# Plachtaa/FAcodec

Measured on AMD Instinct MI355X. Metric: 24kHz audio sec encoded+decoded per wall-sec, higher is better.
Workload: dtype f32; 1 GPU; configs[1]: batch=32/GPU x 2 s @ 24 kHz, forward encoder->FVQ(6 codebooks)->decoder, FAcodec configs/config.yml model (137.7 M params), weights formula-generated, weight-norm re-materialised every step; clips_per_gpu=32, samples_per_clip=48000, parallelism=dp1 (independent clips, no collective)

## Files before the change

facodec_amd/_lib.py:

```python
import ctypes as C
import os

_HERE = os.path.dirname(os.path.abspath(__file__))
LIB_PATH = os.environ.get("FAC_LIB_PATH", os.path.join(_HERE, "libfacodec_hip.so"))

PAD_ZERO, PAD_REFLECT = 0, 1
ACT_NONE, ACT_TANH, ACT_MISH, ACT_LOG_MEL = 0, 1, 2, 3
ACT_GATE, ACT_WN_RES_SKIP = 4, 5

_p = C.c_void_p
_i = C.c_int
_i64 = C.c_int64
_f = C.c_float


class ConvDesc(C.Structure):
    _fields_ = [
        ("x", _p), ("w", _p), ("bias", _p), ("alpha_in", _p), ("alpha_out", _p), ("res", _p), ("y", _p), ("y2", _p), ("alpha_y2", _p), ("w_k1", _p), ("bias_k1", _p),
        ("x_bs", _i64), ("x_cs", _i64), ("y_bs", _i64), ("y_cs", _i64),
        ("B", C.c_int32), ("C_in", C.c_int32), ("T_in", C.c_int32), ("C_out", C.c_int32),
        ("C_out_pad", C.c_int32), ("T_out", C.c_int32),
        ("K", C.c_int32), ("stride", C.c_int32), ("dilation", C.c_int32), ("pad_left", C.c_int32),
        ("pad_mode", C.c_int32), ("n_phase", C.c_int32), ("y_tstride", C.c_int32), ("phase_shift", C.c_int32),
        ("act", C.c_int32),
        ("w_batched", C.c_int32), ("w_bs", _i64), ("ws", _p), ("ws_bytes", _i64), ("w_split", _p),
        ("K1", C.c_int32), ("dilation2", C.c_int32), ("row_phases", C.c_int32),
        ("x_p8", _p), ("x_p8_plane_bytes", _i64), ("y2_p8", _p), ("y2_p8_plane_bytes", _i64),
        ("pw_split", C.c_int32), ("split_rows", C.c_int32),
        ("gate_cond", _p), ("gate_cond_bs", _i64),
        ("keep_tile160", C.c_int32),
    ]


class VqDesc(C.Structure):
    _fields_ = [
        ("residual", _p), ("z_in", _p), ("zq_acc", _p), ("zq_out", _p), ("w_in", _p), ("b_in", _p),
        ("codebook", _p), ("w_out", _p), ("w_out_scale", _p), ("b_out", _p), ("mask", _p), ("codes", _p), ("z_e", _p),
        ("loss_part", _p), ("codes_bs", _i64),
        ("B", C.c_int32), ("D", C.c_int32), ("T", C.c_int32), ("Kc", C.c_int32),
    ]



VQ_DECODE_MAX_Q = 16


class VqDecodeDesc(C.Structure):
    _fields_ = [
        ("codes", _p * 3), ("codes_bs", _i64 * 3), ("codes_qs", _i64 * 3), ("n_q", C.c_int32 * 3),
        ("codebook", _p * VQ_DECODE_MAX_Q), ("w_out", _p * VQ_DECODE_MAX_Q), ("w_out_scale", _p * VQ_DECODE_MAX_Q),
        ("b_out", _p * VQ_DECODE_MAX_Q), ("style", _p), ("outs", _p), ("z", _p * 3),
        ("B", C.c_int32), ("D", C.c_int32), ("T", C.c_int32), ("Kc", C.c_int32),
    ]


class VqDecodeMaskedDesc(C.Structure):
    _fields_ = [("base", VqDecodeDesc), ("n_use", _p), ("n_use_bs", _i64), ("n_use_ts", _i64)]


PLC_MAX_FRAMES = 16
PLC_PRIMARY, PLC_REDUNDANT, PLC_LOST = 0, 1, 2


class PlcSelectDesc(C.Structure):
    _fields_ = [
        ("prim", _p * 3), ("prim_bs", _i64 * 3), ("prim_qs", _i64 * 3),
        ("red", _p * 3), ("red_bs", _i64 * 3), ("red_qs", _i64 * 3),
        ("dst", _p * 3), ("dst_bs", _i64 * 3), ("dst_qs", _i64 * 3),
        ("n_q", C.c_int32 * 3), ("n_red", C.c_int32 * 3),
        ("status", _p), ("last_codes", _p), ("last_n", _p), ("g", _p), ("run", _p),
        ("n_use", _p), ("n_use_bs", _i64), ("n_use_ts", _i64), ("ramp", _p),
        ("B", C.c_int32), ("k", C.c_int32), ("hold", C.c_int32), ("fade", C.c_int32), ("recover", C.c_int32),
        ("reserved", C.c_int32),
    ]


class CodesPackDesc(C.Structure):
    _fields_ = [
        ("codes", _p * 3), ("codes_bs", _i64 * 3), ("codes_qs", _i64 * 3), ("n_q", C.c_int32 * 3),
        ("lens", _p), ("out", _p), ("out_bs", _i64),
        ("B", C.c_int32), ("T", C.c_int32), ("bits", C.c_int32),
    ]


class CodesUnpackDesc(C.Structure):
    _fields_ = [
        ("in_", _p), ("in_bs", _i64), ("codes", _p * 3), ("codes_bs", _i64 * 3), ("codes_qs", _i64 * 3), ("n_q", C.c_int32 * 3),
        ("lens", _p),
        ("B", C.c_int32), ("T", C.c_int32), ("bits", C.c_int32),
    ]


class ResampleDesc(C.Structure):
    _fields_ = [
        ("hist", _p), ("x", _p), ("lens", _p), ("y", _p), ("hist_out", _p), ("table", _p), ("offs", _p),
        ("hist_bs", _i64), ("x_bs", _i64), ("y_bs", _i64), ("q0", _i64), ("m_lo", _i64),
        ("B", C.c_int32), ("n_hist", C.c_int32), ("T", C.c_int32), ("n_out", C.c_int32),
        ("o", C.c_int32), ("n", C.c_int32), ("taps", C.c_int32),
    ]


class KweightDesc(C.Structure):
    _fields_ = [
        ("x", _p), ("lens", _p), ("e", _p), ("state_in", _p), ("state_out", _p), ("peak", _p), ("ws", _p),
        ("x_bs", _i64), ("e_bs", _i64),
        ("B", C.c_int32), ("T", C.c_int32), ("S", C.c_int32), ("offset", C.c_int32), ("peak_accumulate", C.c_int32),
        ("reserved", C.c_int32),
        ("coef", C.c_double * 10), ("pw", C.c_double * 16 * 7),
    ]


SI_SDR_CHUNK = 4096


class StoiDesc(C.Structure):
    _fields_ = [
        ("x", _p), ("y", _p), ("lens", _p), ("kept_idx", _p), ("n_frames", _p), ("n_kept", _p), ("n_segments", _p),
        ("stoi", _p), ("estoi", _p), ("ws", _p),
        ("x_bs", _i64), ("y_bs", _i64), ("ws_bytes", _i64),
        ("B", C.c_int32), ("T", C.c_int32),
    ]


SLOT_MAX_DST, SLOT_TILE = 8, 4096


class SlotSeg(C.Structure):
    _fields_ = [
        ("base", _p), ("slot_hi", _i64),
        ("rows", C.c_int32), ("row_stride", C.c_int32), ("row_len", C.c_int32), ("slot_lo", C.c_int32),
        ("elems", C.c_int32), ("reserved", C.c_int32),
    ]


SIGNATURES = {
    "fac_version": (_i, []),
    "fac_last_error": (C.c_char_p, []),
    "fac_wn_scale": (_i, [_p, _p, _p, _i, _i, _p]),
    "fac_pack_conv_w": (_i, [_p, _p, _p, _i, _i, _i, _i, _p]),
    "fac_pack_convtr_w_rows": (_i, [_p, _p, _p, _i, _i, _i, _p]),
    "fac_conv_w_split_bytes": (_i64, [_i, _i, _i]),
    "fac_conv_w_split2_bytes": (_i64, [_i, _i, _i, _i]),
    "fac_pack_conv_w_split2": (_i, [_p, _p, _p, _i, _i, _i, _i, _p]),
    "fac_gemm_w_split_bytes": (_i64, [_i, _i, _i, _i]),
    "fac_pack_gemm_w_split": (_i, [_p, _i64, _i64, _i64, _p, _p, _i, _i, _i, _i, _p]),
    "fac_pack_conv_w_split": (_i, [_p, _p, _p, _i, _i, _i, _p]),
    "fac_conv_w_split_rows_bytes": (_i64, [_i, _i, _i, _i]),
    "fac_pack_conv_w_split_rows": (_i, [_p, _p, _p, _i, _i, _i, _i, _p]),
    "fac_flip_transpose_w": (_i, [_p, _p, _p, _i, _i, _i, _p]),
    "fac_prep_begin": (_i, []),
    "fac_prep_set_phase": (_i, [_i]),
    "fac_prep_abort": (_i, []),
    "fac_prep_end": (_i, []),
    "fac_prep_replay": (_i, [_i, _p]),
    "fac_prep_info": (_i, [_i, _p, _p]),
    "fac_prep_free": (_i, [_i]),
    "fac_pack_conv_w_bwd": (_i, [_p, _p, _p, _i, _i, _i, _i, _p]),
    "fac_pad_fold_bwd": (_i, [_p, _p, _i, _i, _i, _i, _i, _i, _p]),
    "fac_conv1d_bwd_weight_ws_bytes": (_i64, [_i, _i, _i, _i, _i]),
    "fac_conv1d_bwd_weight": (_i, [_p, _p, _p, _p, _i64, _i, _i, _i, _i, _i, _i, _i, _i, _i, _i, _i, _i, _p]),
    "fac_conv1d_bwd_weight_split_ws_bytes": (_i64, [_i, _i, _i, _i, _i, _i, _i, _i, _i, _i]),
    "fac_conv1d_bwd_weight_split_form": (_i, [_i, _i, _i, _i, _i, _i, _i, _i, _i, _i, _i, C.POINTER(C.c_int)]),
    "fac_conv1d_bwd_weight_k1_ws_bytes": (_i64, [_i, _i, _i, _i]),
    "fac_conv1d_bwd_weight_k1_ws_bytes_for": (_i64, [_p, _p, _i, _i, _i, _i]),
    "fac_conv1d_bwd_weight_taps_tx": (_i64, [_i, _i, _i, _i, _i]),
    "fac_conv1d_bwd_weight_taps_ws_bytes": (_i64, [_i, _i, _i, _i, _i, _i, _i, _i]),
    "fac_conv1d_bwd_weight_taps_ws_bytes_for": (_i64, [_p, _i, _i, _i, _i, _i, _i, _i, _i]),
    "fac_conv1d_bwd_weight_taps": (_i, [_p, _p, _p, _p, _p, _i64, _i, _i, _i, _i, _i, _i, _i, _i, _i, _p]),
    "fac_conv1d_bwd_weight_k1": (_i, [_p, _p, _p, _p, _p, _i64, _i, _i, _i, _i, _p]),
    "fac_conv1d_bwd_weight_split": (_i, [_p, _p, _p, _p, _i64, _i, _i, _i, _i, _i, _i, _i, _i, _i, _i, _i, _i, _p]),
    "fac_conv1d_bwd_weight_split_db_ok": (_i, [_i, _i, _i, _i, _i, _i, _i, _i, _i, _i]),
    "fac_conv1d_bwd_weight_split_db": (_i, [_p, _p, _p, _p, _p, _i64, _i, _i, _i, _i, _i, _i, _i, _i, _i, _i, _i, _i, _p]),
    "fac_weight_norm_bwd": (_i, [_p, _p, _p, _p, _p, _i, _i, _p]),
    "fac_snake_bwd": (_i, [_p, _p, _p, _p, _p, _p, _i, _i, _i, _p]),
    "fac_pack_lstm_whh_t": (_i, [_p, _p, _i, _p]),
    "fac_lstm_layer_bwd": (_i, [_p, _p, _p, _p, _p, _p, _i, _i, _i, _p]),
    "fac_to_p8": (_i, [_p, _p, _p, _i, _i, _i, _p]),
    "fac_lstm_persist_ok": (_i, [_i, _i]),
    "fac_lstm_persist_stream_ok": (_i, [_p]),
    "fac_pack_lstm_whh16": (_i, [_p, _p, _i, _i, _p]),
    "fac_lstm_layer_fwd_persist": (_i, [_p, _p, _p, _p, _p, _p, _i, _i, _i, _i, _p]),
    "fac_lstm_layer_bwd_persist": (_i, [_p, _p, _p, _p, _p, _p, _i, _i, _i, _i, _p]),
    "fac_lstm_persist_split_ok": (_i, [_i, _i]),
    "fac_lstm_persist_timeouts": (_i, []),
    "fac_lstm_persist_arm": (_i, [_p]),
    "fac_lstm_abort_flag": (_i, [_p, _p]),
    "fac_mask_flags_if": (_i, [_p, _i, _p, _p]),
    "fac_pack_lstm_whh_split": (_i, [_p, _p, _i, _p]),
    "fac_lstm_layer_fwd_persist_split": (_i, [_p, _p, _p, _p, _i, _i, _i, _i, _p]),
    "fac_snake_bwd_fused": (_i, [_p, _p, _p, _p, _p, _p, _p, _p, _i, _i, _i, _p]),
    "fac_bias_grad": (_i, [_p, _p, _p, _i, _i, _i, _p]),
    "fac_snake_bwd_fused_rs": (_i, [_p, _p, _p, _i64, _p, _p, _p, _p, _p, _i, _i, _i, _p]),
    "fac_pad_fold_edges": (_i, [_p, _i, _i, _i, _i, _i, _p]),
    "fac_pack_convtr_w": (_i, [_p, _p, _p, _i, _i, _i, _i, _p]),
    "fac_conv1d_fwd": (_i, [C.POINTER(ConvDesc), _p]),
    "fac_conv1d_variant": (_i, [C.POINTER(ConvDesc), C.c_char_p, _i]),
    "fac_snake_fwd": (_i, [_p, _p, _p, _i, _i, _i, _p]),
    "fac_lstm_to_time_major": (_i, [_p, _p, _i, _i, _i, _p]),
    "fac_lstm_from_time_major": (_i, [_p, _p, _p, _p, _i, _i, _i, _p]),
    "fac_pack_lstm_whh": (_i, [_p, _p, _i, _p]),
    "fac_lstm_layer_fwd": (_i, [_p, _p, _p, _p, _i, _i, _i, _p]),
    "fac_lstm_layer_fwd_from": (_i, [_p, _p, _p, _p, _i, _i, _i, _i64, _p]),
    "fac_lstm_layer_fwd_train": (_i, [_p, _p, _p, _p, _p, _p, _i, _i, _i, _i64, _p]),
    "fac_lstm_gate_bwd": (_i, [_p, _p, _p, _p, _p, _p, _p, _i, _i, _i64, _i, _p]),
    "fac_tanh_bwd": (_i, [_p, _p, _p, _i64, _p]),
    "fac_pair_bwd": (_i, [_p, _p, _p, _i64, _i, C.c_float, C.c_float, _i, _p]),
    "fac_spec_power_bwd": (_i, [_p, _p, _p, _i, _i, _i, _i, _p]),
    "fac_stft_frames_bwd": (_i, [_p, _p, _i, _i, _i, _i, _i, _i, _i, _p]),
    "fac_vq_latent_bwd": (_i, [_p, _p, _p, _i64, _p, _p, _p, _p, _i, _i, _p]),
    "fac_vq_codebook_grad": (_i, [_p, _p, _p, _i64, _p, _p, _i, _i, _i, _i, _p]),
    "fac_layernorm_c_affine_bwd": (_i, [_p, _p, _p, _p, _p, _p, _i, _i, _i, _p]),
    "fac_rows_fma": (_i, [_p, _p, _p, _p, _i, _i64, _f, _p]),
    "fac_grad_norm_clip": (_i, [_p, _i64, _f, _p, _p, _p]),
    "fac_adamw_step": (_i, [_p, _p, _p, _p, _i64, _f, _f, _f, _f, _f, _i64, _p, _p]),
    "fac_logdiff_rms_bwd": (_i, [_p, _p, _p, _i, _i, _i, _f, _f, _i, _p]),
    "fac_gather_copy": (_i, [_p, _p, _p, _i, _p]),
    "fac_adamw_step_masked": (_i, [_p, _p, _p, _p, _i64, _p, _i, _p, _p, _p, _f, _f, _f, _f, _f, _p, _p]),
    "fac_gate_bwd": (_i, [_p, _p, _p, _i, _i, _i, _p]),
    "fac_mish_fwd": (_i, [_p, _p, _i64, _p]),
    "fac_mish_bwd": (_i, [_p, _p, _p, _i64, _p]),
    "fac_glu_bwd": (_i, [_p, _p, _p, _i, _i, _i, _p]),
    "fac_mul_scaled": (_i, [_p, _p, _p, _f, _i64, _p]),
    "fac_embed_sum_bwd": (_i, [_p, _p, _p, _i, _i, _i, _i, _i, _i, _i, _p]),
    "fac_gate_bwd_cond": (_i, [_p, _p, _i64, _p, _p, _p, _i64, _i, _i, _i, _p]),
    "fac_masked_mean_bwd": (_i, [_p, _p, _p, _i, _i, _i, _p]),
    "fac_attention_probs": (_i, [_p, _p, _p, _p, _i, _i, _i, _i, _p]),
    "fac_attention_pv": (_i, [_p, _p, _p, _i, _i, _i, _i, _p]),
    "fac_attention_bwd_pv": (_i, [_p, _p, _p, _p, _p, _i, _i, _i, _i, _p]),
    "fac_attention_bwd_qk": (_i, [_p, _p, _p, _p, _p, _p, _p, _i, _i, _i, _i, _p]),
    "fac_aa_snakebeta_bwd": (_i, [_p, _p, _p, _p, _p, _p, _p, _p, _p, _i, _i, _i, _p]),
    "fac_leaky_relu": (_i, [_p, _p, _p, _i64, _f, _i, _i, _i, _i, _i, _p]),
# ... 107 lines not shown
```

facodec_amd/build.py:

```python
import os
import subprocess
import sys
from concurrent.futures import ThreadPoolExecutor

HERE = os.path.dirname(os.path.abspath(__file__))
CSRC = os.path.join(HERE, "csrc")
TAG = os.environ.get("FAC_BUILD_TAG", "")
LIB = os.path.join(HERE, "libfacodec_hip%s.so" % ("_" + TAG if TAG else ""))
OBJDIR = "build" + ("_" + TAG if TAG else "")
SOURCES = ["conv1d_api.hip", "conv1d_tile_128x128.hip", "conv1d_tile_96x128.hip", "conv1d_tile_64x128.hip",
           "conv1d_tile_32x256.hip", "conv1d_tile_128x32.hip", "conv1d_tile_128x256.hip", "conv1d_fused_ru.hip", "conv1d_narrow.hip", "conv1d_pw.hip", "conv1d_pw_split.hip", "conv1d_skinny.hip", "conv1d_bsplit.hip", "conv1d_bsplit96.hip", "conv1d_gemm_split.hip", "conv1d_bsplit2.hip", "conv1d_bwd.hip", "conv1d_wgrad_split.hip", "conv1d_wgrad_k1.hip", "train_misc.hip", "optim.hip", "train_quant.hip", "train_pred.hip", "train_disc.hip", "train_redecoder.hip", "pack.hip", "prep_batch.hip", "lstm.hip", "lstm_persist.hip", "vq.hip", "vq_decode.hip", "bitpack.hip", "misc.hip", "attention_stream.hip", "attention_tiled.hip","ragged.hip", "resample.hip", "loudness.hip", "metrics.hip", "stream_pool.hip", "plc.hip", "jdc.hip", "rccl_arena.hip"]
FLAGS = ["--offload-arch=gfx950", "-O3", "-std=c++17", "-fPIC", "-ffp-contract=off",
         "-Wno-unused-result"] + os.environ.get("FAC_EXTRA_FLAGS", "").split()


def _hipcc():
    for cand in (os.environ.get("HIPCC"), "/opt/rocm/bin/hipcc", "hipcc"):
        if cand and (os.path.isabs(cand) and os.path.exists(cand) or not os.path.isabs(cand)):
            return cand
    return "hipcc"


def _stale(target, deps):
    if not os.path.exists(target):
        return True
    tt = os.path.getmtime(target)
    return any(os.path.getmtime(d) > tt for d in deps)


def build_lib(force=False, verbose=True):
    hipcc = _hipcc()
    headers = sorted(os.path.join(CSRC, f) for f in os.listdir(CSRC) if f.endswith(".h")) + [os.path.join(HERE, "..", "include", "facodec_hip.h")]
    objs, jobs = [], []
    os.makedirs(os.path.join(CSRC, OBJDIR), exist_ok=True)
    for src in SOURCES:
        s = os.path.join(CSRC, src)
        o = os.path.join(CSRC, OBJDIR, src.replace(".hip", ".o"))
        objs.append(o)
        if force or _stale(o, [s] + headers):
            jobs.append([hipcc, *FLAGS, "-c", s, "-o", o])

    def run(cmd):
        if verbose:
            print(" ".join(cmd), file=sys.stderr)
        subprocess.run(cmd, check=True)

    with ThreadPoolExecutor(max_workers=min(8, max(1, len(jobs)))) as ex:
        list(ex.map(run, jobs))
    if force or jobs or _stale(LIB, objs):
        run([hipcc, "--offload-arch=gfx950", "-shared", "-fPIC", *objs, "-ldl", "-o", LIB])
    return LIB


if __name__ == "__main__":
    build_lib(force="--force" in sys.argv)
    print(LIB)
```

facodec_amd/convplan.py:

```python
from collections import namedtuple

__all__ = ["ConvPlan", "ConvTrPlan", "plan_conv", "plan_convtr", "plan_gemm", "tile_rows", "gemm_split_ok", "gemm_split_strided_ok", "split2_ok",
           "pw_taps_ok", "pw_split_tail_ok", "convtr_split_ok", "convtr_rows_ok", "flat_strided_ok", "flat_convtr_ok", "W_FP32", "W_TAPS",
           "W_GEMM", "W_GEMM_STRIDED", "W_SPLIT2", "W_FP32_PW_TAPS", "PER_CLIP", "FLAT_STRIDED", "FLAT_STRIDE1", "TR_POLYPHASE", "TR_ROWS",
           "TR_ROWS_SPLIT", "TR_ROWS_PW_TAPS", "TR_FLAT"]

W_FP32, W_TAPS, W_GEMM, W_GEMM_STRIDED, W_SPLIT2, W_FP32_PW_TAPS = "fp32", "split_taps", "split_gemm", "split_gemm_strided", "split2", "fp32_pw_taps"
PER_CLIP, FLAT_STRIDED, FLAT_STRIDE1 = "per_clip", "flat_strided", "flat_stride1"
ConvPlan = namedtuple("ConvPlan", "layout form p8")
TR_POLYPHASE, TR_ROWS, TR_ROWS_SPLIT, TR_ROWS_PW_TAPS, TR_FLAT = "polyphase", "rows", "rows_split", "rows_pw_taps", "flat_rows_split"
ConvTrPlan = namedtuple("ConvTrPlan", "layout p8")


def _sw():
    from . import ops
    return ops


def gemm_split_ok(c_out, c_in, k, n_cols, t_out=None):
    sw = _sw()
    if not (sw.BF16_SPLIT and k in (1, 2)):
        return False
    if c_in < sw.GEMM_SPLIT_MIN_CIN or c_out < 64 or n_cols < 1024:
        return False
    return k == 1 or (t_out is not None and t_out >= 256)


def gemm_split_strided_ok(c_out, c_in, k, stride, batch, t_out):
    return (_sw().BF16_SPLIT and 1 < stride <= 16 and stride < k <= 2 * stride and c_in >= 32
            and c_out >= 64 and t_out >= 256 and batch * t_out >= 1024)


def split2_ok(c_out, k, k1, stride, n_cols):
    kv = k1 if 0 < k1 < k else k
    return (_sw().BF16_SPLIT and 8 <= c_out <= 32 and ((kv == 9 and stride in (1, 2)) or (kv == 3 and stride == 1))
            and n_cols >= 4096)


def pw_split_tail_ok(c_in, c_out, cols):
    sw = _sw()
    return sw.BF16_SPLIT and sw.PW_SPLIT and c_in == c_out and c_in in (256, 384) and cols >= 65536


def pw_taps_ok(c_in, c_out, k, stride, transposed, batch, t_out):
    sw = _sw()
    if not (sw.BF16_SPLIT and sw.PW_SPLIT and sw.PW_TAPS and stride == 2):
        return False
    taps, rows = (2, 2 * c_out) if transposed else (4, c_out)
    if k != 4 or (c_in * taps) % 64 or c_in * taps > 384 or rows % 64:
        return False
    return batch * ((t_out + 31) // 32) >= 2 * (256 // (rows // 64)) * 12


def convtr_rows_ok(t_in, stride, causal=True):
    sw = _sw()
    return sw.CONVTR_ROWS and causal and 2 <= stride <= 16 and t_in >= sw.CONVTR_ROWS_MIN_T


def convtr_split_ok(c_in, c_out, stride, batch, t_in, causal=True, alpha_in=None):
    return (_sw().BF16_SPLIT and causal and alpha_in is None and 2 <= stride <= 16 and c_in >= 64
            and t_in >= 256 and batch * t_in >= 1024 and c_out * stride >= 64)


def flat_strided_ok(c_out, c_in, k, s, batch, n_out):
    return (_sw().FLAT_TRAIN and k == 2 * s and s > 1 and n_out < 256 and not gemm_split_strided_ok(c_out, c_in, k, s, batch, n_out)
            and gemm_split_strided_ok(c_out, c_in, k, s, 1, batch * (n_out + 1) - 1))


def flat_convtr_ok(c_in, c_out, s, batch, t_cols):
    return (_sw().FLAT_TRAIN and t_cols < 256 and not convtr_split_ok(c_in, c_out, s, batch, t_cols)
            and convtr_split_ok(c_in, c_out, s, 1, batch * t_cols))


def tile_rows(c_out, c_in, k, grad=False):
    sw = _sw()
    return 96 if (sw.BF16_SPLIT and not grad and k == 7 and c_out in sw.BS_ROWS96 and c_in % 8 == 0) else 64


def plan_conv(c_out, c_in, k, stride, dilation, batch, t_in, t_out, *, k1=0, alpha_in=False, plain=True, res=False,
              causal_reflect=False, grad=True, c_out_mult16=True, split_k=(1, 3, 5, 7), floor_k=(3, 5), tail="pw_split",
              pw_taps=True, split2=False, flat_infer=False, flat_stride1=False, flat_train=None):
    sw = _sw()
    cols = batch * t_out
    p8 = 2.0 * c_out * k / (4.0 * stride)
    if split2 and split2_ok(c_out, k, k1, stride, cols):
        return ConvPlan(W_SPLIT2, PER_CLIP, None)
    if stride > 1:
        strided = not alpha_in and dilation == 1 and not k1
        flat_t = (flat_train is not None and strided and plain and t_in % stride == 0
                  and (flat_train == "zero" or (causal_reflect and t_in > stride))
                  and flat_strided_ok(c_out, c_in, k, stride, batch, t_out))
        if flat_t and flat_train == "reflect":
            return ConvPlan(W_GEMM_STRIDED, FLAT_STRIDED, p8)
        if pw_taps and stride == 2 and strided and plain and pw_taps_ok(c_in, c_out, k, 2, False, batch, t_out):
            return ConvPlan(W_FP32_PW_TAPS, PER_CLIP, None)
        if strided and gemm_split_strided_ok(c_out, c_in, k, stride, batch, t_out):
            return ConvPlan(W_GEMM_STRIDED, PER_CLIP, p8)
        if flat_t:
            return ConvPlan(W_GEMM_STRIDED, FLAT_STRIDED, p8)
        if (flat_infer and strided and not res and causal_reflect and k == 2 * stride and t_in % stride == 0 and t_in > stride
                and not grad and gemm_split_strided_ok(c_out, c_in, k, stride, 1, batch * (t_in // stride + 1) - 1)):
            return ConvPlan(W_GEMM_STRIDED, FLAT_STRIDED, p8)
    elif not alpha_in and not k1 and k in split_k:
        if k == 1 and gemm_split_ok(c_out, c_in, 1, cols):
            if not (pw_split_tail_ok(c_in, c_out, cols) if tail == "pw_split"
                    else tail is not None and c_in == c_out and c_in in (256, 384) and cols >= 65536):
                return ConvPlan(W_GEMM, PER_CLIP, None)
        if (sw.BF16_SPLIT and k in (3, 5, 7) and c_in % 16 == 0 and c_out > 2 and (c_out % 16 == 0 or not c_out_mult16)
                and cols > 640 and (k not in floor_k or (c_in >= 64 and c_out > 32))):
            if (flat_infer and flat_stride1 and k == 7 and not res and causal_reflect and not grad and batch >= 4
                    and (k - 1) * dilation < t_in <= 224 and c_in * c_out >= 1 << 20):
                return ConvPlan(W_TAPS, FLAT_STRIDE1, None)
            return ConvPlan(W_TAPS, PER_CLIP, None)
    return ConvPlan(W_FP32, PER_CLIP, None)


def plan_gemm(c_out, c_in, n_cols):
    ok = gemm_split_ok(c_out, c_in, 1, n_cols)
    return ConvPlan(W_GEMM if ok else W_FP32, PER_CLIP, 2.0 * c_out / 4.0 if ok else None)


def plan_convtr(c_in, c_out, stride, batch, t_in, *, causal=True, alpha_in=False, grad=True, flat_infer=False, flat_train_cols=None):
    a = True if alpha_in else None
    p8 = 2.0 * c_out * 2 * stride / 4.0
    if causal and flat_train_cols is not None and flat_convtr_ok(c_in, c_out, stride, batch, flat_train_cols):
        return ConvTrPlan(TR_FLAT, p8)
    if causal and not alpha_in and pw_taps_ok(c_in, c_out, 2 * stride, stride, True, batch, t_in):
        return ConvTrPlan(TR_ROWS_PW_TAPS, None)
    if convtr_split_ok(c_in, c_out, stride, batch, t_in, causal, a):
        return ConvTrPlan(TR_ROWS_SPLIT, p8)
    if flat_infer and not grad and t_in < 256 and convtr_split_ok(c_in, c_out, stride, 1, batch * (t_in + 1), causal, a):
        return ConvTrPlan(TR_FLAT, p8)
    return ConvTrPlan(TR_ROWS if convtr_rows_ok(t_in, stride, causal) else TR_POLYPHASE, None)
```

facodec_amd/csrc/conv1d_api.hip:

```cpp
#include "conv1d_mfma.h"
#include <stdlib.h>

namespace fac {

enum ConvKernel : int {
  CK_128x32 = 0,
  CK_32x256 = 1,
  CK_64x128 = 2,
  CK_96x128 = 3,
  CK_128x128 = 4,
  CK_128x256 = 5,
  CK_96x256 = 6,
  CK_FUSED_RU = 7,
  CK_128x160 = 8,
  CK_NARROW = 9,
  CK_SKINNY = 10,
  CK_BSPLIT = 11,
  CK_CIN1 = 12,
  CK_THIN = 13,
  CK_PW = 14,
  CK_GSPLIT = 15,
  CK_BSPLIT2 = 16,
  CK_PWS = 17,
  CK_PWT = 18,
  CK_BSPLIT96 = 19,
};

static ConvKernel select_variant(const fac_conv_desc* d) {
  const int co = d->C_out;
  if (d->row_phases > 1) return CK_128x256;
  if (d->T_out <= 32) return CK_128x32;
  if (co <= 32) return CK_32x256;
  if (co <= 64) return CK_64x128;
  const bool wide = d->K == 1 && d->n_phase == 1 && d->T_out >= 512;
  if (d->T_out > 128 && d->T_out <= 160 && co > 64) {
    const long long wide_tiles = (long long)d->B * ((co + 127) / 128);
    if (d->K == 1 && d->stride == 1 && d->n_phase == 1 && !d->keep_tile160 && wide_tiles < 256) return CK_128x32;
    return CK_128x160;
  }
  if (co % 128 != 0 && co % 96 == 0) return wide ? CK_96x256 : CK_96x128;
  return wide ? CK_128x256 : CK_128x128;
}

static bool narrow_ok(const fac_conv_desc* d) {
  return d->C_out <= 2 && d->stride == 1 && d->n_phase == 1 && d->phase_shift == 0 && d->y_tstride == 1 && !d->res && !d->y2 &&
         !d->w_batched && d->y && (long long)d->B <= 65535 && (long long)d->B * ((d->T_out + 1023) / 1024) >= 128;
}

static bool pw_enabled() {
  static const bool on = !(getenv("FAC_PW") && getenv("FAC_PW")[0] == '0');
  return on;
}

static int conv_plan(const fac_conv_desc* d, ConvArgs& a, ConvKernel& k) {
  FAC_REQUIRE(d && (d->x || d->x_p8) && (d->w || d->w_split) && (d->y || d->y2 || d->y2_p8), "conv1d: null pointer");
  FAC_REQUIRE(!d->y2 || d->alpha_y2 || d->act == FAC_ACT_WN_RES_SKIP, "conv1d: y2 needs alpha_y2");
  FAC_REQUIRE(d->B > 0 && d->C_in > 0 && d->C_out > 0 && d->T_in > 0 && d->T_out > 0,
              "conv1d: bad shape B=%d C_in=%d C_out=%d T_in=%d T_out=%d", d->B, d->C_in, d->C_out,
              d->T_in, d->T_out);
  FAC_REQUIRE(d->K >= 1 && d->stride >= 1 && d->dilation >= 1 && d->pad_left >= 0,
              "conv1d: bad K/stride/dilation/pad");
  FAC_REQUIRE(d->C_out_pad % 32 == 0 && (d->C_out_pad >= d->C_out || d->row_phases > 1), "conv1d: C_out_pad must be a multiple of 32");
  FAC_REQUIRE(d->n_phase >= 1 && d->y_tstride >= 1, "conv1d: bad phase config");
  FAC_REQUIRE((long long)d->B * d->n_phase <= 65535, "conv1d: B*n_phase too large for grid.z");
  a.x = d->x; a.w = d->w; a.bias = d->bias; a.alpha_in = d->alpha_in; a.alpha_out = d->alpha_out;
  a.res = d->res; a.y = d->y; a.y2 = d->y2; a.alpha2 = d->alpha_y2;
  a.w1 = d->w_k1; a.bias1 = d->bias_k1;
  a.x_p8 = reinterpret_cast<const unsigned char*>(d->x_p8); a.x_p8_ps = d->x_p8_plane_bytes;
  a.y2_p8 = reinterpret_cast<unsigned char*>(d->y2_p8); a.y2_p8_ps = d->y2_p8_plane_bytes;
  FAC_REQUIRE(!d->y2_p8 || d->alpha_y2, "conv1d: y2_p8 needs alpha_y2");
  if (d->w_k1) {
    FAC_REQUIRE(d->C_in == d->C_out && d->C_out_pad == d->C_out && d->n_phase == 1 && d->stride == 1 &&
                    d->alpha_out && d->act == FAC_ACT_NONE && !d->w_batched,
                "conv1d: fused ResidualUnit needs C_in == C_out (multiple of 32), stride 1, a Snake alpha_out");
  }
  a.x_bs = d->x_bs; a.x_cs = d->x_cs; a.y_bs = d->y_bs; a.y_cs = d->y_cs; a.w_bs = d->w_bs;
  a.B = d->B; a.C_in = d->C_in; a.T_in = d->T_in; a.C_out = d->C_out; a.C_out_pad = d->C_out_pad;
  a.T_out = d->T_out; a.K = d->K; a.stride = d->stride; a.dil = d->dilation;
  a.pad_left = d->pad_left; a.pad_mode = d->pad_mode; a.n_phase = d->n_phase;
  a.y_tstride = d->y_tstride; a.act = d->act; a.w_batched = d->w_batched;
  a.phase_shift = d->phase_shift;
  a.rp = d->row_phases > 1 ? d->row_phases : 1;
  FAC_REQUIRE(!d->gate_cond || (d->act == FAC_ACT_GATE && d->gate_cond_bs >= 0),
              "conv1d: gate_cond is the conditioning row of the FAC_ACT_GATE epilogue (act=%d gate_cond_bs=%lld)", d->act,
              (long long)d->gate_cond_bs);
  a.gate_cond = d->gate_cond; a.gate_cond_bs = d->gate_cond_bs;
  if (a.rp > 1) {
    FAC_REQUIRE(d->n_phase == 1 && d->y_tstride == 1 && d->phase_shift == 0 && d->stride == 1 && a.rp <= 128 && !d->w_k1 &&
                    !d->w_batched && d->C_out_pad == fac_convtr_rows(d->C_out, a.rp) && !(d->K1 > 0 && d->K1 < d->K),
                "conv1d: row_phases needs a plain stride-1 launch on weights from fac_pack_convtr_w_rows");
  }
  a.K1 = d->K1 > 0 ? d->K1 : d->K; a.dil2 = d->dilation2;
  FAC_REQUIRE(a.K1 <= d->K && d->K % a.K1 == 0 && (a.K1 == d->K || d->dilation2 > 0), "conv1d: bad two-level taps (K=%d K1=%d)", d->K, d->K1);
  FAC_REQUIRE(!conv_two_level(a) || (!d->w_k1 && d->n_phase == 1 && d->pad_mode == FAC_PAD_ZERO && !d->w_batched),
              "conv1d: two-level taps need a plain, zero-padded conv");
  conv_set_virtual(a);
  FAC_REQUIRE(d->phase_shift >= 0 && d->phase_shift < d->n_phase + (d->n_phase == 1), "conv1d: bad phase_shift");
  {
    long long last = (long long)(d->T_out - 1) * d->stride + (long long)conv_max_tap_offset(a) - d->pad_left;
    int pad_right = last >= d->T_in ? (int)(last - d->T_in + 1) : 0;
    int max_pad = d->pad_left > pad_right ? d->pad_left : pad_right;
    a.T_ext = d->T_in > max_pad ? d->T_in : max_pad + 1;
  }
  if (d->x_p8 || d->y2_p8) {
    const bool gs = d->w_split && (d->K <= 2 || (d->stride > 1 && d->K <= 2 * d->stride)) && conv_gsplit_ok(a) &&
                    !conv_skinny_ok(a, d->ws, d->ws_bytes) && d->C_in % 8 == 0 && d->x_p8_plane_bytes < (1ll << 32);
    const bool ok = !d->y2_p8 && (gs || (d->w_split && !conv_two_level(a) && (d->split_rows == 96 ? conv_bsplit96_p8_ok(a) : conv_bsplit_p8_ok(a)) &&
                                       !conv_cin1_ok(a)));
    FAC_REQUIRE(ok, "conv1d: P8 operands given but the launch does not run on a kernel that takes them (K=%d stride=%d C_in=%d columns=%lld)",
                d->K, d->stride, d->C_in, (long long)d->B * d->T_out);
  }
  if (d->act == FAC_ACT_GATE || d->act == FAC_ACT_WN_RES_SKIP) {
    FAC_REQUIRE(d->w && !d->w_k1 && !d->x_p8 && !conv_two_level(a) && conv_skinny_ok(a, d->ws, d->ws_bytes),
                "conv1d: FAC_ACT_GATE / FAC_ACT_WN_RES_SKIP exist only for few-column launches (B * T_out <= 640) with a workspace");
    k = CK_SKINNY;
    return FAC_OK;
  }
  if (d->w_k1) { k = CK_FUSED_RU; return FAC_OK; }
  a.gflat = 0;
  a.grt = 0;
  if (d->w_split && (a.KV == 9 || a.KV == 3) && d->C_out <= 32 && conv_bsplit2_ok(a)) {
    a.w = reinterpret_cast<const float*>(d->w_split);
    k = CK_BSPLIT2;
    return FAC_OK;
  }
  FAC_REQUIRE(!conv_two_level(a) || d->w, "conv1d: two-level taps outside the split kernel's shapes need fp32 weights");
  const bool pw_on = pw_enabled();
  if (pw_on && d->pw_split && d->w && conv_pwt_ok(a)) { k = CK_PWT; return FAC_OK; }
  if (d->w_split && (d->K <= 2 || (d->stride > 1 && d->K <= 2 * d->stride)) && conv_gsplit_ok(a) &&
      !conv_skinny_ok(a, d->ws, d->ws_bytes)) {
    a.w = reinterpret_cast<const float*>(d->w_split);
    k = CK_GSPLIT;
    return FAC_OK;
  }
  if (a.rp > 1) {
    FAC_REQUIRE(d->w != nullptr && d->w != (const float*)d->w_split, "conv1d: row_phases launch outside the split kernel's shapes needs fp32 weights");
    k = CK_128x256;
    return FAC_OK;
  }
  const bool two_level = conv_two_level(a);
  FAC_REQUIRE(d->split_rows == 0 || d->split_rows == 64 || d->split_rows == 96, "conv1d: split_rows must be 0, 64 or 96");
  if (d->split_rows == 96) {
    FAC_REQUIRE(d->w_split && !two_level && conv_bsplit96_ok(a) && !conv_cin1_ok(a),
                "conv1d: split_rows = 96 needs a stride-1 k = 7 launch with C_out %% 96 == 0, C_in %% 8 == 0 and more than 640 columns "
                "(K=%d stride=%d C_in=%d C_out=%d columns=%lld)", d->K, d->stride, d->C_in, d->C_out, (long long)d->B * d->T_out);
    a.w = reinterpret_cast<const float*>(d->w_split);
    k = CK_BSPLIT96;
    return FAC_OK;
  }
  if (d->w_split && !two_level && conv_bsplit_ok(a) && !conv_cin1_ok(a)) {
    a.w = reinterpret_cast<const float*>(d->w_split);
    k = CK_BSPLIT;
    return FAC_OK;
  }
  FAC_REQUIRE(d->w != nullptr && (const void*)d->w != d->w_split,
              "conv1d: shape does not qualify for a split-bf16 kernel (K=%d stride=%d C_in=%d C_out=%d columns=%lld) and no fp32 "
              "weights were given", d->K, d->stride, d->C_in, d->C_out, (long long)d->B * d->T_out);
  if (!two_level && conv_skinny_ok(a, d->ws, d->ws_bytes)) k = CK_SKINNY;
  else if (narrow_ok(d) && (!two_level || (a.KV - 1) * a.dil <= 64)) k = CK_NARROW;
  else if (conv_thin_ok(a, d->ws, d->ws_bytes)) k = CK_THIN;
  else if (conv_cin1_ok(a)) k = CK_CIN1;
  else if (pw_on && d->pw_split && conv_pw_ok(a) && conv_pws_ok(a)) k = CK_PWS;
  else if (pw_on && conv_pw_ok(a)) k = CK_PW;
  else k = select_variant(d);
  return FAC_OK;
}

}

extern "C" int fac_conv1d_fwd(const fac_conv_desc* d, fac_stream_t stream) {
  using namespace fac;
  ConvArgs a;
  ConvKernel k;
  if (const int rc = conv_plan(d, a, k)) return rc;
  hipStream_t s = (hipStream_t)stream;
  switch (k) {
    case CK_128x32: return conv_dispatch_128x32(a, s);
    case CK_32x256: return conv_dispatch_32x256(a, s);
    case CK_64x128: return conv_dispatch_64x128(a, s);
    case CK_96x128: return conv_dispatch_96x128(a, s);
    case CK_128x128: return conv_dispatch_128x128(a, s);
    case CK_128x256: return conv_dispatch_128x256(a, s);
    case CK_96x256: return conv_dispatch_96x256(a, s);
    case CK_FUSED_RU: return conv_dispatch_fused_ru(a, s);
    case CK_128x160: return conv_dispatch_128x160(a, s);
    case CK_NARROW: return conv_dispatch_narrow(a, s);
    case CK_SKINNY: return conv_dispatch_skinny(a, d->ws, d->ws_bytes, s);
    case CK_BSPLIT: return conv_dispatch_bsplit(a, s);
    case CK_CIN1: return conv_dispatch_cin1(a, s);
    case CK_THIN: return conv_dispatch_thin(a, d->ws, s);
    case CK_PW: return conv_dispatch_pw(a, s);
    case CK_GSPLIT: return conv_dispatch_gsplit(a, s);
    case CK_BSPLIT2: return conv_dispatch_bsplit2(a, s);
    case CK_PWS: return conv_dispatch_pws(a, s);
    case CK_PWT: return conv_dispatch_pwt(a, s);
    case CK_BSPLIT96: return conv_dispatch_bsplit96(a, s);
  }
  return FAC_ERR_ARG;
}

extern "C" int fac_conv1d_variant(const fac_conv_desc* d, char* name, int name_len) {
  using namespace fac;
  ConvArgs a;
  ConvKernel k;
  if (const int rc = conv_plan(d, a, k)) return rc;
  if (!name || name_len <= 0) return k;
  switch (k) {
    case CK_128x32: snprintf(name, name_len, "conv1d_mfma_kernel<1,1,4,1,K> 128x32"); break;
    case CK_32x256: snprintf(name, name_len, "conv1d_mfma_kernel<1,2,1,4,K> 32x256"); break;
    case CK_64x128: snprintf(name, name_len, "conv1d_mfma_kernel<2,1,1,4,K> 64x128"); break;
    case CK_96x128: snprintf(name, name_len, "conv1d_mfma_kernel<3,1,1,4,K> 96x128"); break;
    case CK_128x128: snprintf(name, name_len, "conv1d_mfma_kernel<2,2,2,2,K> 128x128"); break;
    case CK_128x256:
      snprintf(name, name_len, a.rp > 1 ? "conv1d_mfma_kernel<2,2,2,4,2> 128x256 (convtr, all phases per tile)" : "conv1d_mfma_kernel<2,2,2,4,K> 128x256");
      break;
    case CK_96x256: snprintf(name, name_len, "conv1d_mfma_kernel<3,1,1,8,K> 96x256"); break;
    case CK_FUSED_RU: snprintf(name, name_len, "conv1d_mfma_kernel<C/32,1,1,4,7,fused RU> Cx128"); break;
    case CK_128x160: snprintf(name, name_len, "conv1d_mfma_kernel<1,5,4,1,K> 128x160"); break;
    case CK_NARROW:
      snprintf(name, name_len, conv_two_level(a) ? "conv1d_narrow_kernel (VALU, C_out<=2, two-level taps)" : "conv1d_narrow_kernel (VALU, C_out<=2)");
      break;
    case CK_SKINNY:
      snprintf(name, name_len, conv_skinny_single_launch(a) ? "conv1d_gemv_kernel (single launch, <=4 columns)"
                                                            : "conv1d_skinny_kernel (split reduction, <=640 columns)");
      break;
    case CK_BSPLIT: snprintf(name, name_len, "conv1d_bsplit_kernel<%d> 64x256 (bf16x3 split, fp32-grade)", a.K); break;
    case CK_CIN1: snprintf(name, name_len, "conv1d_cin1_kernel (VALU, C_in=1, store stream)"); break;
    case CK_THIN: snprintf(name, name_len, "conv1d_thin_kernel (VALU, C_out<=8, split channels)"); break;
    case CK_PW: snprintf(name, name_len, "conv1d_pw_kernel (k=1 streaming, W in LDS)"); break;
    case CK_GSPLIT:
      snprintf(name, name_len, "conv1d_gemm_split_kernel<%d> 128x128 (bf16x3 split GEMM, fp32-grade)", a.stride > 1 ? 2 : a.K);
      break;
    case CK_BSPLIT2: snprintf(name, name_len, "conv1d_bsplit2_kernel<%d,%d> 32x512 (bf16x3 split, fp32-grade)", a.KV, a.stride); break;
    case CK_PWS: snprintf(name, name_len, "conv1d_pws_kernel (k=1 streaming, W planes in LDS, bf16x3 split, fp32-grade)"); break;
    case CK_PWT: snprintf(name, name_len, "conv1d_pwt_kernel<%d taps> (streaming, W planes in LDS, bf16x3 split, fp32-grade)", a.K); break;
    case CK_BSPLIT96: snprintf(name, name_len, "conv1d_bsplit_kernel<%d> 96x256 (bf16x3 split, fp32-grade)", a.K); break;
  }
  return k;
}
```

facodec_amd/csrc/conv1d_bsplit_kernel.h:

```cpp
#pragma once
#include "conv1d_mfma.h"
#include <type_traits>
#include "inflight_regs.h"
#include "prep_batch.h"

namespace fac {

constexpr int BS_CO = 64;
constexpr int BS96_CO = 96;
constexpr int BS_NSW = 4;
constexpr int BS_NSW_WIDE = 4;
constexpr int BS_XU = 3;
constexpr int BS_WIDE_MIN = 64;
__host__ __device__ constexpr int bs_group(int C_in) { return C_in >= BS_WIDE_MIN ? 2 : 1; }

__host__ __device__ constexpr int bs_slots(int K, int G) { return (G * K + 1) & ~1; }

struct EpiRow {
  float bs, al, inv, a2, i2;
};
__device__ __forceinline__ EpiRow epi_row_load(bool valid, int co, const float* bias, const float* alpha, const float* alpha2) {
  EpiRow r = {0.f, 0.f, 0.f, 0.f, 0.f};
  if (valid) {
    if (bias) r.bs = bias[co];
    if (alpha) { r.al = alpha[co]; r.inv = snake_inv(r.al); }
    if (alpha2) { r.a2 = alpha2[co]; r.i2 = snake_inv(r.a2); }
  }
  return r;
}
__device__ __forceinline__ float epi_row_get(float mine, int lane, int j) {
  return __int_as_float(__builtin_amdgcn_ds_bpermute(((lane & 48) + j) << 2, __float_as_int(mine)));
}

template <int KT, int G, int NMW, int NSW, int MB = 2>
__global__ __launch_bounds__((NMW + NSW) * 64, (NMW + NSW) / 4) void conv1d_bsplit_kernel(ConvArgs a) {
  constexpr int NB = 2;
  constexpr int CO = 32 * MB;
  constexpr bool WIDE = NMW == 4;
  constexpr int BS_TT = 64 * NMW;
  constexpr int H = bs_slots(KT, G);
  constexpr int W_STAGE = 3 * H * CO * 16;
  extern __shared__ __attribute__((aligned(16))) unsigned char sm[];
  const int tid = threadIdx.x;
  const int lane = tid & 63;
  const int wave = __builtin_amdgcn_readfirstlane(tid >> 6);
  const int XW = a.XW;
  const int X_STAGE = 48 * G * XW;
  const int STG = W_STAGE + X_STAGE;
  unsigned char* Wbuf = sm;
  unsigned char* Xbuf = sm + W_STAGE;
  const int n_chunks = (a.C_in + 8 * G - 1) / (8 * G);
  const int dil = a.dil;

  const int n_tiles = a.n_tiles;
  typedef const __attribute__((address_space(4))) ConvArgs* KArgP;
  const KArgP kargs = (KArgP)__builtin_amdgcn_kernarg_segment_ptr();
  auto fresh_args = [&]() {
    KArgP q = kargs;
    asm volatile("" : "+s"(q));
    return q;
  };
  auto decode = [&](KArgP ka, int v, int& t0_, int& co0_, int& b_) {
    const int id = xcd_contiguous_id(v, n_tiles);
    const int nt = ka->n_t_tiles;
    const int tt = id % nt;
    const int rest = id / nt;
    const int nb = ka->B;
    b_ = rest % nb;
    co0_ = (rest / nb) * CO;
    t0_ = tt * BS_TT;
  };
  const bool overlap = a.persist != 0;
  unsigned char* epi_base = sm + (overlap ? STG : 0);
  auto walk = [&](auto role) {
  constexpr int ROLE = decltype(role)::value;
  constexpr bool STAGING = ROLE != 0;
  bool first = true;
  unsigned cboff[BS_XU] = {}, nboff[BS_XU] = {};
  unsigned long long cmask[BS_XU] = {}, nmask[BS_XU] = {};
  const float *cxg = nullptr, *nxg = nullptr;
  const unsigned char *cws = nullptr, *nws = nullptr;
  for (int vb = blockIdx.x; vb < n_tiles; vb += gridDim.x) {
  int t0, co0, b;
  decode(fresh_args(), vb, t0, co0, b);
  const bool has_nt = overlap && vb + (int)gridDim.x < n_tiles;

  if constexpr (STAGING) {
    const int lw = wave - NMW;
    __builtin_amdgcn_s_setprio(FAC_PRIO_STAGE);
    const float* xg = a.x + (long long)b * a.x_bs;
    const int xcs = (int)a.x_cs;
    const unsigned char* wsrc = reinterpret_cast<const unsigned char*>(a.w) + (long long)(co0 / CO) * n_chunks * W_STAGE;
    const int n_blk = (XW + 63) >> 6;
    int u_g[BS_XU], u_c[BS_XU], u_idx[BS_XU];
#pragma unroll
    for (int j = 0; j < BS_XU; ++j) {
      const int u = lw + NSW * j;
      u_g[j] = u % G;
      const int c = (u / G) * 64 + lane;
      u_c[j] = (u < G * n_blk && c < XW) ? c : -1;
      const int tin = t0 - a.pad_left + c;
      int idx;
      if (a.pad_mode == FAC_PAD_REFLECT) idx = reflect_index(tin, a.T_in, a.T_ext);
      else idx = (tin >= 0 && tin < a.T_in) ? tin : -1;
      u_idx[j] = u_c[j] >= 0 ? idx : -1;
    }
    constexpr int NBLK = W_STAGE / 1024;
    constexpr int ND = (NBLK + NSW - 1) / NSW;
    constexpr int NX = BS_XU * 8;
    static_assert(W_STAGE % 1024 == 0 && ND + NX <= 63 && NX == 24, "vmcnt is a 6-bit counter; FAC_XREGS24_* list 24 registers per set");
    auto stage_w = [&](int chunk, int buf) {
      constexpr int N16 = W_STAGE / 16;
      const unsigned char* src = wsrc + (long long)chunk * W_STAGE;
      unsigned char* dst = Wbuf + buf * STG;
      for (int i = lw; i * 64 < N16; i += NSW) {
        const int q = i * 64 + lane;
        if (q < N16)
          __builtin_amdgcn_global_load_lds((glb_void_t*)(src + (long long)q * 16), (lds_void_t*)(dst + i * 1024), 16, 0, 0);
      }
    };
    auto write_x = [&](int buf, const float (&xr)[BS_XU][8]) {
      unsigned char* xd = Xbuf + buf * STG;
#pragma unroll
      for (int j = 0; j < BS_XU; ++j) {
        if (u_c[j] < 0) continue;
        bf16x8 h, m, l;
#pragma unroll
        for (int i = 0; i < 8; ++i) {
          __bf16 p0, p1, p2;
          split3_scalar_sub(xr[j][i], p0, p1, p2);
          h[i] = p0; m[i] = p1; l[i] = p2;
        }
        *reinterpret_cast<bf16x8*>(xd + ((0 * G + u_g[j]) * XW + u_c[j]) * 16) = h;
        *reinterpret_cast<bf16x8*>(xd + ((1 * G + u_g[j]) * XW + u_c[j]) * 16) = m;
        *reinterpret_cast<bf16x8*>(xd + ((2 * G + u_g[j]) * XW + u_c[j]) * 16) = l;
      }
    };
    if constexpr (ROLE == 2) {
      typedef float wv4 __attribute__((ext_vector_type(4)));
      const unsigned char* xp = a.x_p8 + (long long)b * (a.C_in / 8) * a.T_in * 16;
      const long long grp_bytes = (long long)a.T_in * 16;
      unsigned u_poff[BS_XU];
      bool any_pad = false;
#pragma unroll
      for (int j = 0; j < BS_XU; ++j) {
        u_poff[j] = (unsigned)(u_idx[j] >= 0 ? u_idx[j] : 0) * 16u;
        any_pad = any_pad || __builtin_amdgcn_ballot_w64(u_c[j] >= 0 && u_idx[j] < 0) != 0;
      }
      for (int c = -1; c < n_chunks; ++c) {
        if (c + 1 < n_chunks) {
          const int buf = (c + 1) & 1;
          wv4 wv[ND], xv[BS_XU][3];
          const unsigned char* src = wsrc + (long long)(c + 1) * W_STAGE;
#pragma unroll
          for (int j = 0; j < ND; ++j) {
            const int bi = min(lw + NSW * j, NBLK - 1);
// ... 231 lines not shown
            __builtin_amdgcn_sched_barrier(0);
          } else {
            asm volatile("s_waitcnt lgkmcnt(0)" ::: "memory");
            __builtin_amdgcn_s_barrier();
            asm volatile("" ::: "memory");
            __builtin_amdgcn_sched_barrier(0);
            if (chunk + 1 < n_chunks) {
              if (cur == 0) ld(buf ^ 1, 0, A[1], Bf[1]); else ld(buf ^ 1, 0, A[0], Bf[0]);
            }
            if (cur == 0) mma(A[0], Bf[0]); else mma(A[1], Bf[1]);
            if (chunk + 1 < n_chunks) interleave();
            __builtin_amdgcn_sched_barrier(0);
          }
        }
      }
    }
    };
    if (MB == 2 && co0 + 32 >= a.C_out) pipeline(std::integral_constant<int, 1>{});
    else pipeline(std::integral_constant<int, MB>{});
  } else {
  for (int chunk = 0; chunk < n_chunks; ++chunk) {
    const int buf = chunk & 1;
    const unsigned char* Wb = Wbuf + buf * STG + (kq * CO + l31) * 16;
    const unsigned char* Xb = Xbuf + buf * STG + (n0 + l31) * 16 + x_lane;
    bf16x8 A[2][MB][3], Bf[1][NB][3];
    auto ldA = [&](int st, bf16x8 (&Ad)[MB][3]) {
#pragma unroll
      for (int p = 0; p < 3; ++p)
#pragma unroll
        for (int m = 0; m < MB; ++m)
          Ad[m][p] = *reinterpret_cast<const bf16x8*>(Wb + ((p * H + 2 * st) * CO + m * 32) * 16);
    };
    auto ldB = [&](int st, bf16x8 (&Bd)[NB][3]) {
      const int xo = st * x_step;
      constexpr int PO[3] = {1, 0, 2};
#pragma unroll
      for (int pi = 0; pi < 3; ++pi)
#pragma unroll
        for (int n = 0; n < NB; ++n)
          Bd[n][PO[pi]] = *reinterpret_cast<const bf16x8*>(Xb + xo + (PO[pi] * G * XW + n * 32) * 16);
    };
#pragma unroll
    for (int st = 0; st < H / 2; ++st) {
      ldB(st, Bf[0]);
      ldA(st, A[0]);
      __builtin_amdgcn_sched_barrier(0);
      constexpr int TA[6] = {1, 2, 0, 1, 0, 0}, TB[6] = {1, 0, 2, 0, 1, 0};
#pragma unroll
      for (int q = 0; q < 6; ++q)
#pragma unroll
        for (int m = 0; m < MB; ++m)
#pragma unroll
          for (int n = 0; n < NB; ++n)
            acc[m][n] = __builtin_amdgcn_mfma_f32_32x32x16_bf16(A[0][m][TA[q]], Bf[0][n][TB[q]], acc[m][n], 0, 0, 0);
      __builtin_amdgcn_sched_barrier(0);
    }
    __syncthreads();
  }
  }
  __builtin_amdgcn_s_setprio(0);
  {
    float* tile = reinterpret_cast<float*>(epi_base);
    constexpr int EP = BS_TT + 4;
    if constexpr (MB == 3) {
      int lane_off = 4 * kq * EP + n0 + l31;
      asm volatile("" : "+v"(lane_off));
      tile += lane_off;
#pragma unroll
      for (int m = 0; m < MB; ++m)
#pragma unroll
        for (int n = 0; n < NB; ++n)
#pragma unroll
          for (int r = 0; r < 16; ++r) tile[(m * 32 + (r & 3) + 8 * (r >> 2)) * EP + n * 32] = acc[m][n][r];
    } else
#pragma unroll
    for (int m = 0; m < MB; ++m)
#pragma unroll
      for (int n = 0; n < NB; ++n)
#pragma unroll
        for (int r = 0; r < 16; ++r)
          tile[(m * 32 + (r & 3) + 8 * (r >> 2) + 4 * kq) * EP + n0 + n * 32 + l31] = acc[m][n][r];
  }
  }
  __syncthreads();

  {
    const KArgP e = fresh_args();
    const float* tile = reinterpret_cast<const float*>(epi_base);
    constexpr int EP = BS_TT + 4;
    constexpr int NTH = (NMW + NSW) * 64;
    constexpr int QPR = BS_TT / 4;
    float* yg = e->y ? e->y + (long long)b * e->y_bs : nullptr;
    float* y2g = e->y2 ? e->y2 + (long long)b * e->y_bs : nullptr;
    const float* rg = e->res ? e->res + (long long)b * e->y_bs : nullptr;
    const bool vec_ok = (e->y_cs & 3) == 0 && (e->y_bs & 3) == 0 && (!yg || (reinterpret_cast<unsigned long long>(e->y) & 15) == 0) &&
                        (!y2g || (reinterpret_cast<unsigned long long>(e->y2) & 15) == 0) &&
                        (!rg || (reinterpret_cast<unsigned long long>(e->res) & 15) == 0);
    static_assert(QPR % 16 == 0 && NTH % 16 == 0 && (CO * QPR) % 64 == 0 && (CO * QPR + NTH - 1) / NTH <= 16, "EpiRow: 16 lanes share a row, <= 16 iterations");
    const int row_l = (tid + NTH * (lane & 15)) / QPR;
    const EpiRow mine = epi_row_load(row_l < CO && co0 + row_l < e->C_out, co0 + row_l, e->bias, e->alpha_out, y2g ? e->alpha2 : nullptr);
    int j = 0;
    for (int q = tid; q < CO * QPR; q += NTH, ++j) {
      const float bs = epi_row_get(mine.bs, lane, j), al = epi_row_get(mine.al, lane, j), inv = epi_row_get(mine.inv, lane, j);
      float a2 = 0.f, i2 = 0.f;
      if (y2g) { a2 = epi_row_get(mine.a2, lane, j); i2 = epi_row_get(mine.i2, lane, j); }
      const int row = q / QPR, tq = q - row * QPR;
      const int co = co0 + row, t = t0 + 4 * tq;
      if (co >= e->C_out || t >= e->T_out) continue;
      const float4 av = *reinterpret_cast<const float4*>(tile + row * EP + 4 * tq);
      f32x2 v[2] = {{av.x, av.y}, {av.z, av.w}};
      const long long o = (long long)co * e->y_cs + t;
      const bool full = vec_ok && t + 3 < e->T_out;
      float rv[4] = {0.f, 0.f, 0.f, 0.f};
      if (rg) {
        if (full) {
          const float4 r4 = *reinterpret_cast<const float4*>(rg + o);
          rv[0] = r4.x; rv[1] = r4.y; rv[2] = r4.z; rv[3] = r4.w;
        } else {
#pragma unroll
          for (int i = 0; i < 4; ++i) rv[i] = t + i < e->T_out ? rg[o + i] : 0.f;
        }
      }
#pragma unroll
      for (int i = 0; i < 2; ++i) {
        f32x2 x = v[i] + bs;
        if (e->alpha_out) x = snake_apply2(x, al, inv);
        if (e->act != FAC_ACT_NONE) { x.x = apply_act_slow(x.x, e->act); x.y = apply_act_slow(x.y, e->act); }
        v[i] = x + (f32x2){rv[2 * i], rv[2 * i + 1]};
      }
      f32x2 w[2] = {};
      if (y2g) {
#pragma unroll
        for (int i = 0; i < 2; ++i) w[i] = snake_apply2(v[i], a2, i2);
      }
      if (full) {
        if (yg) *reinterpret_cast<float4*>(yg + o) = make_float4(v[0].x, v[0].y, v[1].x, v[1].y);
        if (y2g) *reinterpret_cast<float4*>(y2g + o) = make_float4(w[0].x, w[0].y, w[1].x, w[1].y);
      } else {
#pragma unroll
        for (int i = 0; i < 4; ++i) {
          if (t + i >= e->T_out) continue;
          if (yg) yg[o + i] = v[i >> 1][i & 1];
          if (y2g) y2g[o + i] = w[i >> 1][i & 1];
        }
      }
    }
  }
  first = !overlap;
  if (vb + (int)gridDim.x < n_tiles) __syncthreads();
  }
  };
  if (wave >= NMW) {
    if constexpr (WIDE) {
      if (a.x_p8 != nullptr) walk(std::integral_constant<int, 2>{});
      else walk(std::integral_constant<int, 1>{});
    } else {
      walk(std::integral_constant<int, 1>{});
    }
  } else {
    walk(std::integral_constant<int, 0>{});
  }
}

template <int KT, int G, int NMW, int NSW, int MB = 2>
static int bsplit_launch(ConvArgs& a, hipStream_t s) {
  constexpr int H = bs_slots(KT, G), TT = 64 * NMW, CO = 32 * MB;
  a.XW = TT + (H / G - 1) * a.dil;
  const size_t stg = (size_t)3 * H * CO * 16 + (size_t)48 * G * a.XW;
  const size_t epi = (size_t)CO * (TT + 4) * sizeof(float);
  a.n_t_tiles = (a.T_out + TT - 1) / TT;
  const long long n_wg = (long long)a.n_t_tiles * ((a.C_out + CO - 1) / CO) * a.B;
  if (n_wg > 0x7fffffffll) {
    set_error("conv1d: too many workgroups (%lld)", n_wg);
    return FAC_ERR_ARG;
  }
  const int n_chunks = (a.C_in + 8 * G - 1) / (8 * G);
  int cus = device_cus() & ~7;
  a.persist = (NMW == 4 && a.x_p8 == nullptr && n_chunks % 2 == 0 && cus >= 8 && n_wg > cus &&
               stg + (stg > epi ? stg : epi) <= FAC_LDS_MAX) ? 1 : 0;
  size_t lds = a.persist ? stg + (stg > epi ? stg : epi) : (2 * stg > epi ? 2 * stg : epi);
  if (lds > FAC_LDS_MAX) {
    set_error("conv1d(bf16 split): tile needs %zu B of LDS (dil=%d)", lds, a.dil);
    return FAC_ERR_ARG;
  }
  constexpr auto kern = conv1d_bsplit_kernel<KT, G, NMW, NSW, MB>;
  allow_dynamic_lds<kern>();
  a.n_tiles = (int)n_wg;
  hipLaunchKernelGGL(kern, dim3((unsigned)(a.persist ? cus : n_wg)), dim3((NMW + NSW) * 64), lds, s, a);
  return check_launch("conv1d_bsplit");
}

}
```

facodec_amd/csrc/conv1d_mfma.h:

```cpp
#pragma once
#include "common.h"

namespace fac {

typedef __attribute__((address_space(3))) void lds_void_t;
typedef __attribute__((address_space(1))) const void glb_void_t;

constexpr int CONV_XMAX = 6;

struct ConvArgs {
  const float* x;
  const float* w;
  const float* bias;
  const float* alpha_in;
  const float* alpha_out;
  const float* res;
  float* y;
  float* y2;
  const float* alpha2;
  const float* w1;
  const float* bias1;
  long long x_bs, x_cs, y_bs, y_cs, w_bs;
  int B, C_in, T_in, T_ext, C_out, C_out_pad, T_out;
  int K, stride, dil, pad_left, pad_mode;
  int n_phase, y_tstride, act, w_batched;
  int phase_shift;
  int K1, dil2;
  int K2v, KV, CV;
  int cic;
  int XW;
  int XB;
  int XQ, XR;
  int n_t_tiles;
  int n_tiles, persist;
  int x_off;
  int gflat;
  int grt;
  const unsigned char* x_p8;
  long long x_p8_ps;
  unsigned char* y2_p8;
  long long y2_p8_ps;
  int rp;
  const float* gate_cond;
  long long gate_cond_bs;
};

__host__ __device__ inline int conv_max_tap_offset(const ConvArgs& a) {
  const int K1 = (a.K1 > 0 && a.K1 < a.K) ? a.K1 : a.K;
  return (a.K / K1 - 1) * a.dil2 + (K1 - 1) * a.dil;
}
__host__ __device__ inline bool conv_two_level(const ConvArgs& a) { return a.K1 > 0 && a.K1 < a.K; }
inline void conv_set_virtual(ConvArgs& a) {
  a.KV = conv_two_level(a) ? a.K1 : a.K;
  a.K2v = a.K / a.KV;
  a.CV = a.C_in * a.K2v;
}

template <int KT>
struct ConvUnroll {
  static constexpr int UC = (KT == 1) ? 4 : ((KT == 2 || KT == 3) ? 2 : 1);
  static constexpr int CIC = KT == 1 ? 24 : (KT == 2 || KT == 3) ? 16 : (KT >= 4 && KT <= 7) ? 8 : (KT > 7 ? 4 : 0);
};

template <int KT, int T_TILE>
constexpr int conv_cic() {
  return ((KT == 2 || KT == 3) && T_TILE >= 256) ? 8 : ConvUnroll<KT>::CIC;
}

constexpr int CONV_WPE = 4;
template <int MB, int NB, int WM, int WN, int KT, bool FUSE = false>
__global__ __launch_bounds__((WM * WN + 4) * 64, (WM * WN == 4 ? CONV_WPE : 3)) void conv1d_mfma_kernel(ConvArgs a) {
  constexpr int NMW = WM * WN;
  constexpr int CO_TILE = 32 * MB * WM;
  constexpr int T_TILE = 32 * NB * WN;
  constexpr int CO4 = CO_TILE / 4;
  constexpr bool ALLW = (WM * WN == 8) && !FUSE;
  extern __shared__ __attribute__((aligned(16))) float smem[];

  const int tid = threadIdx.x;
  const int lane = tid & 63;
  const int wave = __builtin_amdgcn_readfirstlane(tid >> 6);

  int t0, co0, b, phase;
  {
    const int id = xcd_contiguous_id<unsigned>(blockIdx.x, gridDim.x);
    const int nt = a.n_t_tiles, nbp = a.B * a.n_phase;
    const int tt = id % nt;
    const int rest = id / nt;
    const int bp = rest % nbp;
    const int ct = rest / nbp;
    t0 = tt * T_TILE;
    co0 = ct * CO_TILE;
    b = bp / a.n_phase;
    phase = bp - b * a.n_phase;
  }
  int y_off = phase - a.phase_shift, tap_shift = 0;
  if (y_off < 0) {
    y_off += a.n_phase;
    tap_shift = 1;
  }

  const int K = KT > 0 ? KT : a.KV;
  const int cic = KT > 0 ? conv_cic<KT, T_TILE>() : a.cic;
  const int XW = a.XW, XB = a.XB;
  const int w_stage = cic * K * CO_TILE;
  const int x_stage = cic * XW;
  float* Wbuf = smem;
  float* Xbuf = smem + 2 * w_stage;
  const int n_chunks = (a.CV + cic - 1) / cic;

  if (wave >= NMW) {
    const int lw = wave - NMW;
    __builtin_amdgcn_s_setprio(3);
    const float* xg = a.x + (long long)b * a.x_bs;
    const int w_rows_total = cin_pad_dev(a.C_in) * a.K;
    const float* wg = a.w + (long long)phase * w_rows_total * a.C_out_pad +
                      (a.w_batched ? (long long)b * a.w_bs : 0ll);
    const int tin0 = t0 * a.stride - a.pad_left - a.x_off;
    const bool vec_ok = ((a.x_cs | a.x_bs) & 3) == 0 && ((reinterpret_cast<unsigned long long>(a.x) & 15) == 0);
    const int r_first = lw / XB, cb_first = lw - r_first * XB;
    const int K2v = a.K2v, dil2 = a.dil2;
    const bool x_dma = a.alpha_in == nullptr && vec_ok && tin0 >= 0 && tin0 + (K2v - 1) * dil2 + XW <= a.T_in &&
                       (K2v == 1 || (dil2 & 3) == 0);

    auto stage = [&](int chunk, int buf) {
      {
        const int n4 = cic * K * CO4;
// ... 412 lines not shown
  constexpr int T_TILE = 32 * NB * WN;
  constexpr int UC = ConvUnroll<KT>::UC;
  constexpr int STEP = 2 * UC;
  a.x_off = ((-a.pad_left) % 4 + 4) % 4;
  a.XW = (((T_TILE - 1) * a.stride + (a.KV - 1) * a.dil + 1 + a.x_off + (a.phase_shift > 0 ? 1 : 0)) + 3) & ~3;
  a.XB = (a.XW / 4 + 63) / 64;
  a.XQ = 4 / a.XB;
  a.XR = 4 % a.XB;
  const int per_ci = a.KV * CO_TILE + a.XW;
  int cic;
  if constexpr (KT > 0) {
    cic = conv_cic<KT, T_TILE>();
    if (cic * a.XB > 4 * CONV_XMAX || (size_t)2 * cic * per_ci * sizeof(float) > (WM * WN == 4 ? 80 : 160) * 1024)
      return launch_cfg<MB, NB, WM, WN, 0, FUSE>(a, s);
  } else {
    int lim = 9216 / per_ci;
    const int lim_regs = (4 * CONV_XMAX) / a.XB;
    if (lim > lim_regs) lim = lim_regs;
    if (lim > 32) lim = 32;
    lim = (lim / STEP) * STEP;
    if (lim < STEP) lim = STEP;
    const int cin_r = ((a.CV + STEP - 1) / STEP) * STEP;
    cic = lim < cin_r ? lim : cin_r;
    for (int c = cic; c >= STEP && c * 2 > cic; c -= STEP)
      if (cin_r % c == 0) { cic = c; break; }
    if (cic * a.XB > 4 * CONV_XMAX) {
      set_error("conv1d: receptive field too wide to stage (K=%d stride=%d dil=%d)", a.K, a.stride, a.dil);
      return FAC_ERR_ARG;
    }
  }
  a.cic = cic;
  size_t lds = (size_t)2 * cic * per_ci * sizeof(float);
  if constexpr ((WM * WN == 8) && !FUSE) {
    const size_t epi = (size_t)CO_TILE * (T_TILE + 4) * sizeof(float);
    if (lds < epi) lds = epi;
  }
  if (lds > FAC_LDS_MAX) {
    set_error("conv1d: tile needs %zu B of LDS (K=%d stride=%d dil=%d)", lds, a.K, a.stride, a.dil);
    return FAC_ERR_ARG;
  }
  constexpr auto kern = conv1d_mfma_kernel<MB, NB, WM, WN, KT, FUSE>;
  allow_dynamic_lds<kern>();
  a.n_t_tiles = (a.T_out + T_TILE - 1) / T_TILE;
  if (a.rp > 1 && !((WM * WN == 8) && !FUSE && CO_TILE == 128)) {
    set_error("conv1d: row_phases needs the 128-row all-waves-epilogue tile");
    return FAC_ERR_ARG;
  }
  const int n_co_tiles = a.rp > 1 ? a.C_out_pad / CO_TILE : (a.C_out + CO_TILE - 1) / CO_TILE;
  const long long n_wg = (long long)a.n_t_tiles * n_co_tiles * a.B * a.n_phase;
  if (n_wg > 0x7fffffffll) {
    set_error("conv1d: too many workgroups (%lld)", n_wg);
    return FAC_ERR_ARG;
  }
  hipLaunchKernelGGL(kern, dim3((unsigned)n_wg), dim3((WM * WN + 4) * 64), lds, s, a);
  return check_launch("conv1d_mfma");
}

int conv_dispatch_128x128(ConvArgs& a, hipStream_t s);
int conv_dispatch_96x128(ConvArgs& a, hipStream_t s);
int conv_dispatch_64x128(ConvArgs& a, hipStream_t s);
int conv_dispatch_32x256(ConvArgs& a, hipStream_t s);
int conv_dispatch_128x32(ConvArgs& a, hipStream_t s);
int conv_dispatch_128x256(ConvArgs& a, hipStream_t s);
int conv_dispatch_96x256(ConvArgs& a, hipStream_t s);
int conv_dispatch_fused_ru(ConvArgs& a, hipStream_t s);
int conv_dispatch_128x160(ConvArgs& a, hipStream_t s);
int conv_dispatch_narrow(ConvArgs& a, hipStream_t s);
bool conv_cin1_ok(const ConvArgs& a);
bool conv_pw_ok(const ConvArgs& a);
int conv_dispatch_pw(ConvArgs& a, hipStream_t s);
bool conv_thin_ok(const ConvArgs& a, const void* ws, long long ws_bytes);
int conv_dispatch_thin(ConvArgs& a, void* ws, hipStream_t s);
int conv_dispatch_cin1(ConvArgs& a, hipStream_t s);
bool conv_bsplit2_ok(const ConvArgs& a);
int conv_dispatch_bsplit2(ConvArgs& a, hipStream_t s);
bool conv_gsplit_ok(const ConvArgs& a);
int conv_dispatch_gsplit(ConvArgs& a, hipStream_t s);
bool conv_bsplit_ok(const ConvArgs& a);
bool conv_bsplit_p8_ok(const ConvArgs& a);
int conv_dispatch_bsplit(ConvArgs& a, hipStream_t s);
bool conv_bsplit96_ok(const ConvArgs& a);
bool conv_bsplit96_p8_ok(const ConvArgs& a);
int conv_dispatch_bsplit96(ConvArgs& a, hipStream_t s);
bool conv_pws_ok(const ConvArgs& a);
int conv_dispatch_pws(ConvArgs& a, hipStream_t s);
bool conv_pwt_ok(const ConvArgs& a);
int conv_dispatch_pwt(ConvArgs& a, hipStream_t s);
bool conv_skinny_ok(const ConvArgs& a, const void* ws, long long ws_bytes);
bool conv_skinny_single_launch(const ConvArgs& a);
int conv_dispatch_skinny(ConvArgs& a, void* ws, long long ws_bytes, hipStream_t s);

}
```

facodec_amd/csrc/inflight_regs.h:

```cpp
#pragma once

#define FAC_XREGS24_A(M) M(0, 208) M(1, 209) M(2, 210) M(3, 211) M(4, 212) M(5, 213) M(6, 214) M(7, 215) M(8, 216) M(9, 217) M(10, 218) \
  M(11, 219) M(12, 220) M(13, 221) M(14, 222) M(15, 223) M(16, 224) M(17, 225) M(18, 226) M(19, 227) M(20, 228) M(21, 229) M(22, 230) M(23, 231)
#define FAC_XREGS24_B(M) M(0, 232) M(1, 233) M(2, 234) M(3, 235) M(4, 236) M(5, 237) M(6, 238) M(7, 239) M(8, 240) M(9, 241) M(10, 242) \
  M(11, 243) M(12, 244) M(13, 245) M(14, 246) M(15, 247) M(16, 248) M(17, 249) M(18, 250) M(19, 251) M(20, 252) M(21, 253) M(22, 254) M(23, 255)
#define FAC_XREGS40_A(M) M(0, 176) M(1, 177) M(2, 178) M(3, 179) M(4, 180) M(5, 181) M(6, 182) M(7, 183) M(8, 184) M(9, 185) M(10, 186) \
  M(11, 187) M(12, 188) M(13, 189) M(14, 190) M(15, 191) M(16, 192) M(17, 193) M(18, 194) M(19, 195) M(20, 196) M(21, 197) M(22, 198) M(23, 199) \
  M(24, 200) M(25, 201) M(26, 202) M(27, 203) M(28, 204) M(29, 205) M(30, 206) M(31, 207) M(32, 208) M(33, 209) M(34, 210) M(35, 211) M(36, 212) \
  M(37, 213) M(38, 214) M(39, 215)
#define FAC_XREGS40_B(M) M(0, 216) M(1, 217) M(2, 218) M(3, 219) M(4, 220) M(5, 221) M(6, 222) M(7, 223) M(8, 224) M(9, 225) M(10, 226) \
  M(11, 227) M(12, 228) M(13, 229) M(14, 230) M(15, 231) M(16, 232) M(17, 233) M(18, 234) M(19, 235) M(20, 236) M(21, 237) M(22, 238) M(23, 239) \
  M(24, 240) M(25, 241) M(26, 242) M(27, 243) M(28, 244) M(29, 245) M(30, 246) M(31, 247) M(32, 248) M(33, 249) M(34, 250) M(35, 251) M(36, 252) \
  M(37, 253) M(38, 254) M(39, 255)
```

facodec_amd/csrc/misc.hip:

```cpp
#include "common.h"
#include <string.h>

namespace fac {

static thread_local char g_err[512] = "";

void set_error(const char* fmt, ...) {
  va_list ap;
  va_start(ap, fmt);
  vsnprintf(g_err, sizeof(g_err), fmt, ap);
  va_end(ap);
}

constexpr int EW_THREADS = 256;
inline int ew_grid(long long n, int per_thread = 1) {
  long long g = (n + (long long)EW_THREADS * per_thread - 1) / ((long long)EW_THREADS * per_thread);
  if (g > 8192) g = 8192;
  if (g < 1) g = 1;
  return (int)g;
}

__global__ void snake_kernel(const float* __restrict__ x, const float* __restrict__ alpha,
                             float* __restrict__ y, int C, int T, long long n) {
  for (long long i = (long long)blockIdx.x * blockDim.x + threadIdx.x; i < n;
// ... 487 lines not shown
    int m = 2 * t0 - 5 + i;
    m = m < 0 ? 0 : (m > 2 * T - 1 ? 2 * T - 1 : m);
    float u = 0.f;
    const int ip_lo = (m + 4 + 1) >> 1;
#pragma unroll
    for (int q = 0; q < 6; ++q) {
      const int ip = ip_lo + q;
      const int k = m + 15 - 2 * ip;
      if (k >= 0 && k <= 11) {
        int t = ip - 5;
        t = t < 0 ? 0 : (t > T - 1 ? T - 1 : t);
        u = fmaf(xs[t - (t0 - 8)], f[k], u);
      }
    }
    u = __fmul_rn(2.0f, u);
    const float sn = sin_sq(__fmul_rn(u, ea));
    as[i] = __fadd_rn(u, __fmul_rn(inv, sn));
  }
  __syncthreads();
  const int t = t0 + threadIdx.x;
  if (t < T) {
    float o = 0.f;
#pragma unroll
    for (int j = 0; j < 12; ++j) o = fmaf(as[2 * threadIdx.x + j], f[j], o);
    y[(long long)bc * T + t] = o;
  }
}

__global__ __launch_bounds__(256) void logdiff_rms_stage1(const float* __restrict__ a,
                                                          const float* __restrict__ b,
                                                          float* __restrict__ scratch, int M, int T,
                                                          long long n_cols, float eps) {
  __shared__ float part[4];
  float s = 0.f;
  for (long long i = (long long)blockIdx.x * 256 + threadIdx.x; i < n_cols; i += (long long)gridDim.x * 256) {
    const long long bb = i / T;
    const int t = (int)(i - bb * T);
    const float* pa = a + bb * M * T + t;
    const float* pb = b + bb * M * T + t;
    float q = 0.f;
    for (int m = 0; m < M; ++m) {
      const float d = logf(fabsf(pa[(long long)m * T]) + eps) - logf(fabsf(pb[(long long)m * T]) + eps);
      q = fmaf(d, d, q);
    }
    s += sqrtf(q / (float)M);
  }
#pragma unroll
  for (int o = 32; o > 0; o >>= 1) s += __shfl_down(s, o, 64);
  if ((threadIdx.x & 63) == 0) part[threadIdx.x >> 6] = s;
  __syncthreads();
  if (threadIdx.x == 0) scratch[blockIdx.x] = (part[0] + part[1]) + (part[2] + part[3]);
}

__global__ __launch_bounds__(256) void logdiff_rms_bwd_kernel(const float* __restrict__ a, const float* __restrict__ b,
                                                              float* __restrict__ db, int M, int T, long long n_cols, float eps,
                                                              float scale, int accumulate) {
  for (long long i = (long long)blockIdx.x * 256 + threadIdx.x; i < n_cols; i += (long long)gridDim.x * 256) {
    const long long bb = i / T;
    const int t = (int)(i - bb * T);
    const float* pa = a + bb * M * T + t;
    const float* pb = b + bb * M * T + t;
    float* pd = db + bb * M * T + t;
    float q = 0.f;
    for (int m = 0; m < M; ++m) {
      const float d = logf(fabsf(pa[(long long)m * T]) + eps) - logf(fabsf(pb[(long long)m * T]) + eps);
      q = fmaf(d, d, q);
    }
    const float r = sqrtf(q / (float)M);
    const float k = r > 0.f ? scale / ((float)M * r) : 0.f;
    for (int m = 0; m < M; ++m) {
      const float bv = pb[(long long)m * T];
      const float d = logf(fabsf(pa[(long long)m * T]) + eps) - logf(fabsf(bv) + eps);
      const float sg = bv > 0.f ? 1.f : (bv < 0.f ? -1.f : 0.f);
      const float g = -k * d * sg / (fabsf(bv) + eps);
      pd[(long long)m * T] = accumulate ? pd[(long long)m * T] + g : g;
    }
  }
}

}

using namespace fac;

extern "C" int fac_version(void) { return 5; }
extern "C" const char* fac_last_error(void) { return fac::g_err; }

#define EW_LAUNCH(kern, n, ...)                                                         \
  hipLaunchKernelGGL(kern, dim3(ew_grid(n)), dim3(EW_THREADS), 0, (hipStream_t)stream, __VA_ARGS__)

extern "C" int fac_snake_fwd(const float* x, const float* alpha, float* y, int B, int C, int T,
                             fac_stream_t stream) {
  FAC_REQUIRE(x && alpha && y && B > 0 && C > 0 && T > 0, "snake_fwd: bad arguments");
  const long long n = (long long)B * C * T;
  if (T >= 1024 && (long long)B * C <= 65535) {
    hipLaunchKernelGGL(snake_rows_kernel, dim3((T + 1023) / 1024, B * C), dim3(256), 0, (hipStream_t)stream, x, alpha, y, C, T);
  } else {
    EW_LAUNCH(snake_kernel, n, x, alpha, y, C, T, n);
  }
  return check_launch("snake_fwd");
}

extern "C" int fac_gate_tanh_sigmoid(const float* a, const float* g, int64_t g_bs, float* out, int B,
                                     int C, int T, fac_stream_t stream) {
  FAC_REQUIRE(a && out && B > 0 && C > 0 && T > 0, "gate_tanh_sigmoid: bad arguments");
  const long long n = (long long)B * C * T;
  EW_LAUNCH(gate_kernel, n, a, g, out, C, T, (long long)g_bs, n);
  return check_launch("gate_tanh_sigmoid");
}

extern "C" int fac_embed_sum(const int64_t* codes, const float* tables, float* out, int B, int n_tab,
                             int n_codes, int code_row0, int V, int E, int T, int accumulate,
                             fac_stream_t stream) {
  FAC_REQUIRE(codes && tables && out && B > 0 && n_tab >= 0 && V > 0 && E > 0 && T > 0 &&
                  code_row0 >= 0 && code_row0 + n_tab <= n_codes, "embed_sum: bad arguments");
  const long long n = (long long)B * E * T;
  EW_LAUNCH(embed_sum_kernel, n, (const long long*)codes, tables, out, n_tab, n_codes, code_row0, V, E, T, n,
            accumulate);
  return check_launch("embed_sum");
}

extern "C" int fac_glu_residual(const float* a, const float* res, float* out, int B, int C, int T,
                                fac_stream_t stream) {
  FAC_REQUIRE(a && res && out && B > 0 && C > 0 && T > 0, "glu_residual: bad arguments");
  const long long n = (long long)B * C * T;
  EW_LAUNCH(glu_res_kernel, n, a, res, out, C, T, n);
  return check_launch("glu_residual");
}

extern "C" int fac_add(const float* a, const float* b, float* out, int64_t n, fac_stream_t stream) {
  FAC_REQUIRE(a && b && out && n > 0, "add: bad arguments");
  EW_LAUNCH(add_kernel, n, a, b, out, (long long)n);
  return check_launch("add");
}

extern "C" int fac_sub2(const float* a, const float* b, const float* c, float* out, int64_t n,
                        fac_stream_t stream) {
  FAC_REQUIRE(a && b && c && out && n > 0, "sub2: bad arguments");
  EW_LAUNCH(sub2_kernel, n, a, b, c, out, (long long)n);
  return check_launch("sub2");
}

extern "C" int fac_mul_mask(float* x, const float* mask, int B, int C, int T, fac_stream_t stream) {
  FAC_REQUIRE(x && mask && B > 0 && C > 0 && T > 0, "mul_mask: bad arguments");
  const long long n = (long long)B * C * T;
  EW_LAUNCH(mul_mask_kernel, n, x, mask, C, T, n);
  return check_launch("mul_mask");
}

extern "C" int fac_stream_push(float* buf, const float* src, int64_t rows, int64_t cap, int hist, int n_prev,
                               int n_new, fac_stream_t stream) {
  FAC_REQUIRE(buf && src && rows > 0 && hist >= 0 && hist <= 2048 && n_prev >= 0 && n_new > 0 &&
                  cap >= (int64_t)hist + n_new && cap >= (int64_t)hist + n_prev,
              "stream_push: bad arguments (rows=%lld cap=%lld hist=%d n_prev=%d n_new=%d)", (long long)rows,
              (long long)cap, hist, n_prev, n_new);
  hipLaunchKernelGGL(stream_push_kernel, dim3((unsigned)rows), dim3(256), 0, (hipStream_t)stream, buf, src,
                     (long long)cap, hist, n_prev, n_new);
  return check_launch("stream_push");
}

extern "C" int fac_wn_res_skip(const float* rs, float* x, float* out, int B, int C, int T, int last,
                               fac_stream_t stream) {
  FAC_REQUIRE(rs && out && (last || x) && B > 0 && C > 0 && T > 0, "wn_res_skip: bad arguments");
  const long long n = (long long)B * C * T;
  EW_LAUNCH(wn_res_skip_kernel, n, rs, x, out, C, T, last, n);
  return check_launch("wn_res_skip");
}

// ... 185 lines not shown
```

facodec_amd/csrc/pack.hip:

```cpp
#include "common.h"
#include "prep_batch.h"

namespace fac {

__device__ __forceinline__ void wn_scale_body(const float* __restrict__ v, const float* __restrict__ g,
                                              float* __restrict__ scale, int slice_len, int vb, float* part) {
  const int i = vb;
  if (g == nullptr) {
    if (threadIdx.x == 0) scale[i] = 1.0f;
    return;
  }
  const float* p = v + (long long)i * slice_len;
  float s = 0.f;
  for (int j = threadIdx.x; j < slice_len; j += 256) {
    float x = p[j];
    s = fmaf(x, x, s);
  }
#pragma unroll
  for (int o = 32; o > 0; o >>= 1) s += __shfl_down(s, o, 64);
  if ((threadIdx.x & 63) == 0) part[threadIdx.x >> 6] = s;
  __syncthreads();
  if (threadIdx.x == 0) {
    float tot = (part[0] + part[1]) + (part[2] + part[3]);
    scale[i] = __fdiv_rn(g[i], sqrtf(tot));
// ... 37 lines not shown
                                                        float* __restrict__ out, int C_out, int R, int C_out_pad, int R_pad) {
  __shared__ float tile[32][33];
  pack_conv_body(v, scale, out, C_out, R, C_out_pad, R_pad, blockIdx.x, blockIdx.y, tile);
}

__device__ __forceinline__ void pack_convtr_body(const float* __restrict__ v, const float* __restrict__ scale,
                                                 float* __restrict__ out, int C_in, int C_out, int s, int C_out_pad,
                                                 int bx, int by, float* tl) {
  const int K = 2 * s;
  const int ci = bx;
  const int c0 = by * 32;
  const bool real = ci < C_in;
  const float sc = (scale && real) ? scale[ci] : 1.0f;
  const float* src = v + ((long long)(real ? ci : 0) * C_out + c0) * K;
  const int n = 32 * K;
  for (int i = threadIdx.x; i < n; i += 256) {
    const int co = i / K, k = i - co * K;
    float val = 0.f;
    if (real && c0 + co < C_out) val = __fmul_rn(src[i], sc);
    tl[co * (K + 1) + k] = val;
  }
  __syncthreads();
  for (int i = threadIdx.x; i < n; i += 256) {
    const int co = i & 31;
    const int pj = i >> 5;
    const int p = pj >> 1, j = pj & 1;
    const int k = p + s * (1 - j);
    if (c0 + co < C_out_pad)
      out[(((long long)p * cin_pad_dev(C_in) + ci) * 2 + j) * C_out_pad + c0 + co] = tl[co * (K + 1) + k];
  }
}

__global__ __launch_bounds__(256) void pack_convtr_kernel(const float* __restrict__ v, const float* __restrict__ scale,
                                                          float* __restrict__ out, int C_in, int C_out, int s, int C_out_pad) {
  extern __shared__ float tl[];
  pack_convtr_body(v, scale, out, C_in, C_out, s, C_out_pad, blockIdx.x, blockIdx.y, tl);
}

__device__ __forceinline__ void pack_convtr_rows_body(const float* __restrict__ v, const float* __restrict__ scale,
                                                      float* __restrict__ out, int C_in, int C_out, int s, int R_pad,
                                                      long long n, int vb, int vg) {
  const int cpt = 128 / s;
  for (long long i = (long long)vb * 256 + threadIdx.x; i < n; i += (long long)vg * 256) {
    const int row = (int)(i % R_pad);
    const long long r2 = i / R_pad;
    const int j = (int)(r2 & 1);
    const int ci = (int)(r2 >> 1);
    const int tile = row >> 7, rl = row & 127;
    const int cl = rl / s, p = rl - cl * s;
    const int co = tile * cpt + cl;
    float val = 0.f;
    if (ci < C_in && cl < cpt && co < C_out) {
      val = v[((long long)ci * C_out + co) * (2 * s) + p + s * (1 - j)];
      if (scale) val = __fmul_rn(val, scale[ci]);
    }
    out[i] = val;
  }
}

__global__ __launch_bounds__(256) void pack_convtr_rows_kernel(const float* __restrict__ v, const float* __restrict__ scale,
                                                               float* __restrict__ out, int C_in, int C_out, int s, int R_pad,
                                                               long long n) {
  pack_convtr_rows_body(v, scale, out, C_in, C_out, s, R_pad, n, blockIdx.x, gridDim.x);
}

__device__ __forceinline__ void flip_transpose_w_body(const float* __restrict__ v, const float* __restrict__ scale,
                                                      float* __restrict__ out, int C_out, int C_in, int K, long long n, int vb, int vg) {
  for (long long i = (long long)vb * 256 + threadIdx.x; i < n; i += (long long)vg * 256) {
    const int k = (int)(i % K);
    const long long r = i / K;
    const int co = (int)(r % C_out);
    const int ci = (int)(r / C_out);
    float w = v[((long long)co * C_in + ci) * K + (K - 1 - k)];
    if (scale) w = __fmul_rn(w, scale[co]);
    out[i] = w;
  }
}

__global__ __launch_bounds__(256) void flip_transpose_w_kernel(const float* __restrict__ v, const float* __restrict__ scale,
                                                               float* __restrict__ out, int C_out, int C_in, int K, long long n) {
  flip_transpose_w_body(v, scale, out, C_out, C_in, K, n, blockIdx.x, gridDim.x);
}

__global__ __launch_bounds__(256) void pack_batch_kernel(const PrepJob* __restrict__ jobs, const int* __restrict__ first, int njobs) {
  __shared__ float sm[32 * 33];
  const int j = prep_find_job(first, njobs, blockIdx.x);
  const PrepJob& J = jobs[j];
  const int vb = blockIdx.x - first[j];
  const float* a = static_cast<const float*>(J.a);
  const float* b = static_cast<const float*>(J.b);
  float* o = static_cast<float*>(J.out);
  switch (J.kind) {
    case PK_WN_SCALE: wn_scale_body(a, b, o, J.i[0], vb, sm); break;
    case PK_CONV: pack_conv_body(a, b, o, J.i[0], J.i[1], J.i[2], J.i[3], vb % J.i[4], vb / J.i[4], reinterpret_cast<float (*)[33]>(sm)); break;
    case PK_CONVTR: pack_convtr_body(a, b, o, J.i[0], J.i[1], J.i[2], J.i[3], vb % J.i[4], vb / J.i[4], sm); break;
    case PK_CONVTR_ROWS: pack_convtr_rows_body(a, b, o, J.i[0], J.i[1], J.i[2], J.i[3], J.n, vb, J.nblocks); break;
    case PK_FLIP_T: flip_transpose_w_body(a, b, o, J.i[0], J.i[1], J.i[2], J.n, vb, J.nblocks); break;
    default: break;
  }
}

int prep_launch_pack(const PrepJob* jobs, const int* first, int njobs, int total, hipStream_t s) {
  hipLaunchKernelGGL(pack_batch_kernel, dim3(total), dim3(256), 0, s, jobs, first, njobs);
  return check_launch("pack_batch");
}

__global__ __launch_bounds__(256) void pack_whh_kernel(const float* __restrict__ w,
                                                       float* __restrict__ out, int H) {
  const long long n = (long long)4 * H * H;
  for (long long o = (long long)blockIdx.x * 256 + threadIdx.x; o < n;
       o += (long long)gridDim.x * 256) {
    const int jj = o & 3;
    const int i = (o >> 2) & 31;
    const int kq = (o >> 7) & 1;
    const long long rest = o >> 8;
    const int kgs = H / 8;
    const int kg = rest % kgs;
    const int ublk = rest / kgs;
    const int gate = i >> 3, u = i & 7;
    const int row = gate * H + ublk * 8 + u;
    const int k = kg * 8 + 2 * jj + kq;
    out[o] = w[(long long)row * H + k];
  }
}

}

extern "C" int fac_wn_scale(const float* v, const float* g, float* scale, int n_slices,
                            int slice_len, fac_stream_t stream) {
  using namespace fac;
  FAC_REQUIRE(scale && n_slices > 0 && slice_len > 0 && (v || !g), "wn_scale: bad arguments");
  if (prep_recording()) {
    PrepJob j{}; j.a = v; j.b = g; j.out = scale; j.kind = PK_WN_SCALE; j.nblocks = n_slices; j.i[0] = slice_len;
    return prep_record(PU_PACK, j);
  }
  hipLaunchKernelGGL(wn_scale_kernel, dim3(n_slices), dim3(256), 0, (hipStream_t)stream, v, g,
                     scale, slice_len);
  return check_launch("wn_scale");
}

extern "C" int fac_pack_conv_w(const float* v, const float* scale, float* packed, int C_out,
                               int C_in, int K, int C_out_pad, fac_stream_t stream) {
  using namespace fac;
  FAC_REQUIRE(v && packed && C_out > 0 && C_in > 0 && K > 0, "pack_conv_w: bad arguments");
  FAC_REQUIRE(C_out_pad % 32 == 0 && C_out_pad >= C_out, "pack_conv_w: C_out_pad must be a multiple of 32");
  const int R = C_in * K;
  const int R_pad = cin_pad_dev(C_in) * K;
  dim3 grid((R_pad + 31) / 32, C_out_pad / 32);
  if (prep_recording()) {
    PrepJob j{}; j.a = v; j.b = scale; j.out = packed; j.kind = PK_CONV; j.nblocks = (int)(grid.x * grid.y);
    j.i[0] = C_out; j.i[1] = R; j.i[2] = C_out_pad; j.i[3] = R_pad; j.i[4] = (int)grid.x;
    return prep_record(PU_PACK, j);
  }
  hipLaunchKernelGGL(pack_conv_kernel, grid, dim3(256), 0, (hipStream_t)stream, v, scale, packed,
                     C_out, R, C_out_pad, R_pad);
  return check_launch("pack_conv_w");
}

extern "C" int fac_pack_convtr_w(const float* v, const float* scale, float* packed, int C_in,
                                 int C_out, int stride, int C_out_pad, fac_stream_t stream) {
  using namespace fac;
  FAC_REQUIRE(v && packed && C_out > 0 && C_in > 0 && stride > 0, "pack_convtr_w: bad arguments");
  FAC_REQUIRE(C_out_pad % 32 == 0 && C_out_pad >= C_out, "pack_convtr_w: C_out_pad must be a multiple of 32");
  dim3 grid(cin_pad_dev(C_in), C_out_pad / 32);
  const size_t lds = (size_t)32 * (2 * stride + 1) * sizeof(float);
  if (prep_recording()) {
    FAC_REQUIRE(2 * stride <= 32, "pack_convtr_w: a recorded launch takes strides up to 16");
    PrepJob j{}; j.a = v; j.b = scale; j.out = packed; j.kind = PK_CONVTR; j.nblocks = (int)(grid.x * grid.y);
    j.i[0] = C_in; j.i[1] = C_out; j.i[2] = stride; j.i[3] = C_out_pad; j.i[4] = (int)grid.x;
    return prep_record(PU_PACK, j);
  }
  hipLaunchKernelGGL(pack_convtr_kernel, grid, dim3(256), lds, (hipStream_t)stream, v, scale,
                     packed, C_in, C_out, stride, C_out_pad);
  return check_launch("pack_convtr_w");
}

extern "C" int fac_pack_convtr_w_rows(const float* v, const float* scale, float* packed, int C_in, int C_out, int stride,
                                      fac_stream_t stream) {
  using namespace fac;
  FAC_REQUIRE(v && packed && C_out > 0 && C_in > 0 && stride > 0 && stride <= 128, "pack_convtr_w_rows: bad arguments");
  const int R_pad = fac_convtr_rows(C_out, stride);
  const long long n = (long long)cin_pad_dev(C_in) * 2 * R_pad;
  const int blocks = (int)((n + 255) / 256 < 65535 ? (n + 255) / 256 : 65535);
  if (prep_recording()) {
    PrepJob j{}; j.a = v; j.b = scale; j.out = packed; j.kind = PK_CONVTR_ROWS; j.nblocks = blocks; j.n = n;
    j.i[0] = C_in; j.i[1] = C_out; j.i[2] = stride; j.i[3] = R_pad;
    return prep_record(PU_PACK, j);
  }
  hipLaunchKernelGGL(pack_convtr_rows_kernel, dim3(blocks), dim3(256), 0, (hipStream_t)stream, v, scale, packed, C_in, C_out,
                     stride, R_pad, n);
  return check_launch("pack_convtr_w_rows");
}

extern "C" int fac_flip_transpose_w(const float* v, const float* scale, float* out, int C_out, int C_in, int K, fac_stream_t stream) {
  using namespace fac;
  FAC_REQUIRE(v && out && C_out > 0 && C_in > 0 && K > 0, "flip_transpose_w: bad arguments");
  const long long n = (long long)C_out * C_in * K;
  const int blocks = (int)((n + 255) / 256 < 65535 ? (n + 255) / 256 : 65535);
  if (prep_recording()) {
    PrepJob j{}; j.a = v; j.b = scale; j.out = out; j.kind = PK_FLIP_T; j.nblocks = blocks; j.n = n;
    j.i[0] = C_out; j.i[1] = C_in; j.i[2] = K;
    return prep_record(PU_PACK, j);
  }
  hipLaunchKernelGGL(flip_transpose_w_kernel, dim3(blocks), dim3(256), 0, (hipStream_t)stream, v, scale, out, C_out, C_in, K, n);
  return check_launch("flip_transpose_w");
}

extern "C" int fac_pack_lstm_whh(const float* w_hh, float* packed, int H, fac_stream_t stream) {
  using namespace fac;
  FAC_REQUIRE(w_hh && packed && H > 0 && H % 8 == 0, "pack_lstm_whh: H must be a multiple of 8");
  hipLaunchKernelGGL(pack_whh_kernel, dim3(2048), dim3(256), 0, (hipStream_t)stream, w_hh, packed, H);
  return check_launch("pack_lstm_whh");
}
```

facodec_amd/csrc/prep_batch.h:

```cpp
#pragma once
#include "common.h"

namespace fac {

struct PrepJob {
  const void* a;
  const void* b;
  void* out;
  long long n;
  long long l[3];
  int kind;
  int nblocks;
  int i[8];
};

enum PrepUnit { PU_PACK = 0, PU_BSPLIT, PU_GSPLIT, PU_BSPLIT2, PU_BWD, PU_COUNT };

enum PrepKind {
  PK_WN_SCALE = 0, PK_CONV, PK_CONVTR, PK_CONVTR_ROWS, PK_FLIP_T,
  PK_CONV_SPLIT,
  PK_GEMM_SPLIT,
  PK_CONV_SPLIT2,
  PK_CONV_BWD
};

bool prep_recording();
int prep_record(int unit, const PrepJob& j);

int prep_launch_pack(const PrepJob* jobs, const int* first, int njobs, int total, hipStream_t s);
int prep_launch_bsplit(const PrepJob* jobs, const int* first, int njobs, int total, hipStream_t s);
int prep_launch_gsplit(const PrepJob* jobs, const int* first, int njobs, int total, hipStream_t s);
int prep_launch_bsplit2(const PrepJob* jobs, const int* first, int njobs, int total, hipStream_t s);
int prep_launch_bwd(const PrepJob* jobs, const int* first, int njobs, int total, hipStream_t s);

inline int prep_blocks(long long n) { return (int)((n + 255) / 256 < 65535 ? (n + 255) / 256 : 65535); }

__device__ __forceinline__ int prep_find_job(const int* __restrict__ first, int njobs, int b) {
  int lo = 0, hi = njobs - 1;
  while (lo < hi) {
    const int mid = (lo + hi + 1) >> 1;
    if (first[mid] <= b) lo = mid; else hi = mid - 1;
  }
  return lo;
}

}
```

facodec_amd/dac_model.py:

```python
from torch import nn

from . import autograd as A
from . import ops
from .wprep import cached_forward
from .layers import SConv1d, SConvTranspose1d, SLSTM, Snake1d, write_edge

FUSED_RU_CHANNELS = (64,)


class ResidualUnit(nn.Module):

    def __init__(self, dim=16, dilation=1, causal=False):
        super().__init__()
        self.block = nn.Sequential(
            Snake1d(dim),
            SConv1d(dim, dim, kernel_size=7, dilation=dilation, causal=causal, norm="weight_norm"),
            Snake1d(dim),
            SConv1d(dim, dim, kernel_size=1, causal=causal, norm="weight_norm"),
        )

    @property
    def alpha_in(self):
        return self.block[0].flat()

    def run(self, x, x_act, alpha_next=None, want_raw=True, edge=None):
        b = self.block
        k7, k1 = b[1], b[3]
        streaming = ops.BF16_SPLIT and x.shape[0] * ((x.shape[-1] + 31) // 32) >= 8192
        if k7.w.c_out in FUSED_RU_CHANNELS and x_act.shape[-1] == x.shape[-1] and not streaming:
            write_edge(k7, x_act, edge)
            return_pair = ops.conv1d(x_act, k7.w.packed(), k7.w.c_out, 7, bias=k7.w.bias, dilation=k7.dilation,
                                     alpha_out=b[2].flat(), res=x, w_k1=k1.w.packed(), bias_k1=k1.w.bias,
                                     alpha_y2=alpha_next, want_y=want_raw or alpha_next is None, causal=k7.causal)
            return return_pair if alpha_next is not None else (return_pair, None)
        h = b[1].run(x_act, alpha_out=b[2].flat(), edge=edge)
        if h.shape[-1] != x.shape[-1]:
            pad = (x.shape[-1] - h.shape[-1]) // 2
            x = x[..., pad:-pad].contiguous()
        if alpha_next is None:
            return b[3].run(h, res=x), None
        return b[3].run(h, res=x, alpha_y2=alpha_next, want_y=want_raw)

    def forward(self, x):
        if self.training:
            b = self.block
            y = A.conv(b[3], A.snake(b[2], A.conv(b[1], A.snake(b[0], x))))
            return A.add(x, y)
        return self.run(x, ops.snake(x, self.alpha_in))[0]


def _run_units(units, x, x_act, alpha_after, edge=None):
    for j, ru in enumerate(units):
        last = j == len(units) - 1
        nxt = alpha_after if last else units[j + 1].alpha_in
        x, x_act = ru.run(x, x_act, alpha_next=nxt, want_raw=not last, edge=edge)
    return x_act


class EncoderBlock(nn.Module):

    def __init__(self, dim=16, stride=1, causal=False):
        super().__init__()
        self.block = nn.Sequential(
            ResidualUnit(dim // 2, dilation=1, causal=causal),
            ResidualUnit(dim // 2, dilation=3, causal=causal),
            ResidualUnit(dim // 2, dilation=9, causal=causal),
            Snake1d(dim // 2),
            SConv1d(dim // 2, dim, kernel_size=2 * stride, stride=stride, causal=causal, norm="weight_norm"),
        )

    @property
    def alpha_in(self):
        return self.block[0].alpha_in

    def run(self, x, x_act, alpha_next=None):
        b = self.block
        z_act = _run_units([b[0], b[1], b[2]], x, x_act, b[3].flat())
        return b[4].run(z_act, alpha_y2=alpha_next) if alpha_next is not None else (b[4].run(z_act), None)

    def forward(self, x):
        return self.run(x, ops.snake(x, self.alpha_in))[0]


class Encoder(nn.Module):

    def __init__(self, d_model=64, strides=(2, 4, 8, 8), d_latent=64, causal=False, lstm=2):
        super().__init__()
        layers = [SConv1d(1, d_model, kernel_size=7, causal=causal, norm="weight_norm")]
        for s in strides:
            d_model *= 2
            layers.append(EncoderBlock(d_model, stride=s, causal=causal))
        self.use_lstm = lstm
        if lstm:
            layers.append(SLSTM(d_model, lstm))
        layers += [Snake1d(d_model), SConv1d(d_model, d_latent, kernel_size=3, causal=causal, norm="weight_norm")]
        self.block = nn.Sequential(*layers)
        self.enc_dim = d_model
        self.boundary_hook = None

    def _forward_train(self, x):
        mods = list(self.block)
        x = A.conv(mods[0], x)
        for m in mods[1:-2]:
            if self.boundary_hook is not None:
                self.boundary_hook(m, x)
            if isinstance(m, EncoderBlock):
                b = m.block
                x, xa = A.snake_dual(x, b[0].block[0].alpha)
                for j in range(3):
                    nxt = b[j + 1].block[0].alpha if j < 2 else b[3].alpha
                    x, xa = A.res_unit(b[j], x, xa, nxt)
                x = A.conv(b[4], xa)
            else:
                x = A.slstm(m, x)
        return A.conv(mods[-1], A.snake(mods[-2], x))

    @cached_forward
# ... 117 lines not shown
```

facodec_amd/layers.py:

```python
import math

import torch
from torch import nn

from . import ops


def _uniform_(t, bound):
    with torch.no_grad():
        return t.uniform_(-bound, bound)


class ConvWeights(nn.Module):

    def __init__(self, c_in, c_out, k, weight_norm=True, transposed=False, stride=1, bias=True):
        super().__init__()
        self.c_in, self.c_out, self.k = c_in, c_out, k
        self.transposed, self.stride, self.weight_norm = transposed, stride, weight_norm
        shape = (c_in, c_out, k) if transposed else (c_out, c_in, k)
        fan_in = (c_out if transposed else c_in) * k
        w = _uniform_(torch.empty(shape), 1.0 / math.sqrt(fan_in))
        if weight_norm:
            self.weight_g = nn.Parameter(w.reshape(shape[0], -1).norm(dim=1).reshape(shape[0], 1, 1))
            self.weight_v = nn.Parameter(w)
        else:
            self.weight = nn.Parameter(w)
        self.bias = nn.Parameter(_uniform_(torch.empty(c_out), 1.0 / math.sqrt(fan_in))) if bias else None
        self._packed = None
        self._split = None
        self._rows = None
        self._rows_split = None
        self.freeze_packed = False

    def _vg(self):
        return (self.weight_v.detach(), self.weight_g.detach()) if self.weight_norm else (self.weight.detach(), None)

    def _cached(self, slot, pack, *a, **kw):
        cur = getattr(self, slot)
        if cur is None or not self.freeze_packed:
            cur = pack(*self._vg(), *a, out=cur[0] if isinstance(cur, tuple) else cur, **kw)
            setattr(self, slot, cur)
        return cur

    def packed(self):
        if self.transposed:
            return self._cached("_packed", ops.pack_convtr_weight, self.stride)
        return self._cached("_packed", ops.pack_conv_weight)

    def packed_rows(self):
        return self._cached("_rows", ops.pack_convtr_weight_rows, self.stride)

    def packed_rows_split(self):
        return self._cached("_rows_split", ops.pack_convtr_weight_rows_split, self.stride)

    def packed_split_strided(self, stride):
        return self._cached("_split", ops.pack_gemm_weight_split, in_stride=stride)

    def packed_split(self, rows=64):
        return self._cached("_split", ops.pack_conv_weight_split, rows=rows)

    def _apply(self, fn, *a, **kw):
        self._packed = None
        self._split = None
        self._rows = None
        self._rows_split = None
        return super()._apply(fn, *a, **kw)


class _Norm(nn.Module):

    def __init__(self, name, weights):
        super().__init__()
        setattr(self, name, weights)


FLAT_SHORT_CLIPS = True
FLAT_STRIDE1 = True


def write_edge(conv, x, edge):
    rule = conv.edge_rule() if edge is not None else None
    if rule is not None:
        ops.edge_tail_(x, edge[0], edge[1], rule[0], rule[1])


class SConv1d(nn.Module):

    def __init__(self, in_channels, out_channels, kernel_size, stride=1, dilation=1, causal=False,
                 norm="none", pad_mode="reflect", bias=True):
        super().__init__()
        self.conv = _Norm("conv", ConvWeights(in_channels, out_channels, kernel_size, norm == "weight_norm", bias=bias))
        self.kernel_size, self.stride, self.dilation = kernel_size, stride, dilation
        self.causal = causal
        self.pad_mode = ops.PAD_REFLECT if pad_mode == "reflect" else ops.PAD_ZERO

    @property
    def w(self):
        return self.conv.conv

    def plan(self, B, T, alpha_in=False, plain=True, res=False):
        return ops.plan_conv(self.w.c_out, self.w.c_in, self.kernel_size, self.stride, self.dilation, B, T, -(-T // self.stride),
                             alpha_in=alpha_in, plain=plain, res=res, causal_reflect=self.causal and self.pad_mode == ops.PAD_REFLECT,
                             grad=torch.is_grad_enabled(), c_out_mult16=False, tail="always", flat_infer=FLAT_SHORT_CLIPS,
                             flat_stride1=FLAT_STRIDE1)

    def edge_rule(self):
        if self.causal:
            return None
        if self.stride != 1:
            raise NotImplementedError(f"a non-causal strided SConv1d (k = {self.kernel_size}, stride {self.stride}) pads its right "
                                      "side by an amount that depends on the clip's length: no per-clip edge rule")
        n = ((self.kernel_size - 1) * self.dilation) // 2
        return (n, self.pad_mode) if n > 0 else None

    def run(self, x, alpha_in=None, alpha_out=None, res=None, act=ops.ACT_NONE, alpha_y2=None, want_y=True, edge=None):
        w, k, s_ = self.w, self.kernel_size, self.stride
        write_edge(self, x, edge)
        B, _, T = x.shape
        plan = self.plan(B, T, alpha_in is not None, alpha_out is None and res is None and act == ops.ACT_NONE, res is not None)
        split = (w.packed_split_strided(s_) if plan.layout == ops.W_GEMM_STRIDED
                 else w.packed_split(ops.tile_rows(w.c_out, w.c_in, k)) if plan.layout == ops.W_TAPS
                 else w.packed_split() if plan.layout == ops.W_GEMM else None)
        if plan.form != ops.PER_CLIP:
            P = (k - 1) * self.dilation + 1 - s_
            return ops.conv1d_flat(torch.nn.functional.pad(x, (P, 0), mode="reflect"), split, w.c_out, k, s_, T // s_,
                                   dilation=self.dilation, bias=w.bias, p8=plan.p8, alpha_out=alpha_out, act=act, alpha_y2=alpha_y2,
                                   want_y=want_y)
        x = ops.p8_prepass(x, plan.p8)
        return ops.conv1d(x, w.packed() if split is None else None, w.c_out, k, bias=w.bias,
                          stride=s_, dilation=self.dilation, pad_mode=self.pad_mode, alpha_in=alpha_in,
                          alpha_out=alpha_out, res=res, act=act, causal=self.causal, alpha_y2=alpha_y2, want_y=want_y,
                          w_split=split)

    def forward(self, x):
        return self.run(x)


class SConvTranspose1d(nn.Module):

    def __init__(self, in_channels, out_channels, kernel_size, stride=1, causal=False, norm="none"):
        super().__init__()
        self.convtr = _Norm("convtr", ConvWeights(in_channels, out_channels, kernel_size, norm == "weight_norm",
                                                  transposed=True, stride=stride))
        self.stride = stride
        self.causal = causal

# ... 80 lines not shown
```

facodec_amd/ops.py:

```python
import ctypes as C
import math
import os
from collections import namedtuple

import torch

from . import _lib
from .wprep import prepared
from .convplan import *
from ._lib import ConvDesc, VqDesc, VqDecodeDesc, ResampleDesc, PAD_REFLECT, PAD_ZERO, ACT_NONE, ACT_TANH, ACT_MISH, ACT_LOG_MEL, ACT_GATE, ACT_WN_RES_SKIP


def pad32(n):
    return (n + 31) & ~31


def cin_pad(c):
    return ((c + 47) // 48) * 48


_RAW_STREAM = getattr(torch._C, "_cuda_getCurrentRawStream", None)
_GET_DEVICE = getattr(torch._C, "_cuda_getDevice", None)


# ... 91 lines not shown
        raise _lib.FacodecHipError(f"ConvTranspose1d needs kernel_size == 2*stride (got {k}, {stride})")
    scale = wn_scale(v, g) if g is not None else None
    if out is None:
        out = torch.empty(cin_pad(c_in), 2, convtr_rows_pad(c_out, stride), device=v.device, dtype=torch.float32)
    _lib.check(_lib.load().fac_pack_convtr_w_rows(_ptr(v), _ptr(scale), _ptr(out), c_in, c_out, stride, _stream()),
               "fac_pack_convtr_w_rows")
    return out


class ConvLaunchProfile:

    def __init__(self):
        self.records = []

    def summary(self):
        out = {}
        for name, flops, e0, e1 in self.records:
            r = out.setdefault(name, dict(launches=0, flops=0.0, ms=0.0))
            r["launches"] += 1
            r["flops"] += flops
            r["ms"] += e0.elapsed_time(e1)
        return out


_PROFILE = None


class FlopCounter:

    def __init__(self):
        self.flops = dict(conv=0.0, wgrad=0.0, lstm=0.0, dft=0.0)
        self.launches = dict(conv=0, wgrad=0, lstm=0, dft=0)

    def add(self, key, f):
        self.flops[key] += f * _FLOP_SCALE
        self.launches[key] += 1

    @property
    def total(self):
        return sum(v for k, v in self.flops.items() if k != "dft")


_FLOPS = None
_FLOP_SCALE = 1.0


def set_flop_counter(c):
    global _FLOPS
    _FLOPS = c


_FLOP_KEY = "conv"


class flop_key:

    def __init__(self, key):
        self.key = key

    def __enter__(self):
        global _FLOP_KEY
        self.prev, _FLOP_KEY = _FLOP_KEY, self.key

    def __exit__(self, *a):
        global _FLOP_KEY
        _FLOP_KEY = self.prev


class flop_scale:

    def __init__(self, s):
        self.s = s

    def __enter__(self):
        global _FLOP_SCALE
        self.prev, _FLOP_SCALE = _FLOP_SCALE, self.s

    def __exit__(self, *a):
        global _FLOP_SCALE
        _FLOP_SCALE = self.prev

BF16_SPLIT = True
BS_ROWS96 = (96,)


def set_conv_profile(p):
    global _PROFILE
    _PROFILE = p


_CONV_WS = {}
CONV_WS_BYTES = 32 << 20


_STREAM_SLOTS = {}


def register_stream_slot(stream):
    key = stream.cuda_stream
    if key not in _STREAM_SLOTS:
        _STREAM_SLOTS[key] = len(_STREAM_SLOTS) + 1
    return _STREAM_SLOTS[key]


_SIDE_STREAMS = {}


def side_streams(device, n):
    key = (device, n)
    if key not in _SIDE_STREAMS:
        _SIDE_STREAMS[key] = [torch.cuda.Stream(device=device) for _ in range(n)]
        for st in _SIDE_STREAMS[key]:
            register_stream_slot(st)
    return _SIDE_STREAMS[key]


def join_side_streams(device):
    if device.type != "cuda":
        return
    cur = torch.cuda.current_stream(device)
    for (dev, _), streams in _SIDE_STREAMS.items():
        if dev.type == "cuda" and (dev.index is None or device.index is None or dev.index == device.index):
            for st in streams:
                if st != cur:
                    cur.wait_stream(st)


def run_chains(chains, device, n_streams, inputs=()):
    n = min(n_streams, len(chains))
    if n <= 1 or device.type != "cuda":
        return [c() for c in chains]
    main = torch.cuda.current_stream(device)
    streams = side_streams(device, n)
    for st in streams:
        st.wait_stream(main)
        _record_stream(inputs, st)
    outs = []
    for j, c in enumerate(chains):
        with torch.cuda.stream(streams[j % n]):
            outs.append(c())
    for st in streams:
        main.wait_stream(st)
    _record_stream(outs, main)
    return outs


def _record_stream(obj, stream):
    if torch.is_tensor(obj):
        if obj.is_cuda:
            obj.record_stream(stream)
    elif isinstance(obj, (list, tuple)):
        for o in obj:
            _record_stream(o, stream)
    elif isinstance(obj, dict):
        for o in obj.values():
            _record_stream(o, stream)


_CUDA_DEVICES = {}


def _cuda_device(index):
    d = _CUDA_DEVICES.get(index)
    if d is None:
        d = _CUDA_DEVICES[index] = torch.device("cuda", index)
    return d


def _conv_workspace(device):
    slot = _STREAM_SLOTS.get(_raw_stream(device.index), 0) if _STREAM_SLOTS else 0
    key = (device, slot)
    ws = _CONV_WS.get(key)
    if ws is None:
        ws = _CONV_WS[key] = torch.zeros(CONV_WS_BYTES // 4, device=device, dtype=torch.float32)
    return ws


def conv_variant(d):
    buf = C.create_string_buffer(96)
    return _lib.load().fac_conv1d_variant(C.byref(d), buf, 96), buf.value.decode()


def _launch_conv(d, what):
    lib = _lib.load()
    ws = _conv_workspace(_cuda_device(_GET_DEVICE() if _GET_DEVICE is not None else torch.cuda.current_device()))
    d.ws, d.ws_bytes = ws.data_ptr(), CONV_WS_BYTES
    if _FLOPS is not None or _PROFILE is not None:
        flops = 2.0 * d.B * d.n_phase * max(1, d.row_phases) * d.C_out * d.T_out * d.C_in * d.K
        if d.w_k1:
            flops += 2.0 * d.B * d.C_out * d.T_out * d.C_out
    if _FLOPS is not None:
        _FLOPS.add(_FLOP_KEY, flops)
    if _PROFILE is None:
        _lib.check(lib.fac_conv1d_fwd(C.byref(d), _stream()), what)
        return
    name = conv_variant(d)[1][:63]
    e0, e1 = torch.cuda.Event(enable_timing=True), torch.cuda.Event(enable_timing=True)
    e0.record()
    _lib.check(lib.fac_conv1d_fwd(C.byref(d), _stream()), what)
    e1.record()
    _PROFILE.records.append((name, flops, e0, e1))


GEMM_SPLIT_MIN_CIN = 256


@prepared
def pack_gemm_weight_split(v, g=None, out=None, in_stride=1, scale=None):
    v = _dev(v, "weight")
    if v.dim() == 2:
        v = v.unsqueeze(-1)
    c_out, c_in, k = v.shape
    lib = _lib.load()
    if scale is None and g is not None:
        scale = wn_scale(v, g)
    nbytes = lib.fac_gemm_w_split_bytes(c_out, c_in, k, in_stride)
    if out is None:
        out = torch.empty(nbytes, device=v.device, dtype=torch.uint8)
    _lib.check(lib.fac_pack_gemm_w_split(_ptr(v), c_in * k, k, 1, _ptr(scale), out.data_ptr(), c_out, c_in, k, in_stride, _stream()),
               "fac_pack_gemm_w_split")
    return out


def pack_gemm_weight_split_t(w, out=None):
    w = _dev(w, "weight")
    if w.dim() == 2:
        w = w.unsqueeze(-1)
    c_out, c_in, k = w.shape
    assert k == 1
    lib = _lib.load()
    nbytes = lib.fac_gemm_w_split_bytes(c_in, c_out, 1, 1)
    if out is None:
        out = torch.empty(nbytes, device=w.device, dtype=torch.uint8)
    _lib.check(lib.fac_pack_gemm_w_split(_ptr(w), 1, c_in, 1, None, out.data_ptr(), c_in, c_out, 1, 1, _stream()),
               "fac_pack_gemm_w_split(transposed)")
    return out


@prepared
def pack_conv_weight_split2(v, g=None, k1=0, out=None, scale=None):
    v = _dev(v, "weight")
    c_out, c_in, k = v.shape
    lib = _lib.load()
    if scale is None and g is not None:
        scale = wn_scale(v, g)
    nbytes = lib.fac_conv_w_split2_bytes(c_out, c_in, k, k1)
    if out is None:
        out = torch.empty(nbytes, device=v.device, dtype=torch.uint8)
    _lib.check(lib.fac_pack_conv_w_split2(_ptr(v), _ptr(scale), out.data_ptr(), c_out, c_in, k, k1, _stream()),
               "fac_pack_conv_w_split2")
    return out


@prepared
def pack_convtr_weight_rows_split(v, g, stride, out=None):
    rows = pack_convtr_weight_rows(v, g, stride)
    cip, _, R = rows.shape
    c_in = v.shape[0]
    lib = _lib.load()
    nbytes = lib.fac_gemm_w_split_bytes(R, c_in, 2, 1)
    if out is None:
        out = torch.empty(nbytes, device=v.device, dtype=torch.uint8)
    _lib.check(lib.fac_pack_gemm_w_split(_ptr(rows), 1, 2 * R, R, None, out.data_ptr(), R, c_in, 2, 1, _stream()),
               "fac_pack_gemm_w_split(convtr rows)")
    return out, R


@prepared
def pack_conv_weight_split(v, g=None, out=None, scale=None, rows=None):
    v = _dev(v, "weight")
    c_out, c_in, k = v.shape
    if k <= 2:
        return pack_gemm_weight_split(v, g, out=out, scale=scale)
    lib = _lib.load()
    if scale is None and g is not None:
        scale = wn_scale(v, g)
    if rows is None:
        rows = tile_rows(c_out, c_in, k)
    nbytes = lib.fac_conv_w_split_rows_bytes(c_out, c_in, k, rows)
    if nbytes < 0:
        raise _lib.FacodecHipError("pack_conv_weight_split: no %d-row tile for k = %d" % (rows, k))
    if out is None or out.numel() != nbytes:
        out = torch.empty(nbytes, device=v.device, dtype=torch.uint8)
    _lib.check(lib.fac_pack_conv_w_split_rows(_ptr(v), _ptr(scale), out.data_ptr(), c_out, c_in, k, rows, _stream()),
               "fac_pack_conv_w_split_rows")
    out.split_rows = rows
    return out


def conv_out_len(t_in, k, stride, dilation):
    k_eff = (k - 1) * dilation + 1
    padding_total = k_eff - stride
    n_frames = (t_in - k_eff + padding_total) / stride + 1
    ideal = (math.ceil(n_frames) - 1) * stride + (k_eff - padding_total)
    extra = ideal - t_in
    t_out = (t_in + padding_total + extra - k_eff) // stride + 1
    return t_out, padding_total, extra


class P8:

    def __init__(self, planes, shape):
        self.planes, self.shape = planes, tuple(shape)

    @staticmethod
    def empty(B, C, T, device):
        return P8(torch.empty(3, B * (C // 8) * T + 1, 8, device=device, dtype=torch.bfloat16), (B, C, T))

    @property
    def plane_bytes(self):
        return self.planes.stride(0) * 2

    def to_float(self):
        B, C, T = self.shape
        v = self.planes[:, :-1].float().sum(0).reshape(B, C // 8, T, 8)
        return v.permute(0, 1, 3, 2).reshape(B, C, T).contiguous()


def to_p8(x, alpha=None):
    x = _dev(x, "x")
    B, C, T = x.shape
    out = P8.empty(B, C, T, x.device)
    _lib.check(_lib.load().fac_to_p8(_ptr(x), _ptr(alpha), _ptr(out.planes), B, C, T, _stream()), "fac_to_p8")
    return out


P8_PREPASS_MIN_FLOP_PER_BYTE = 450.0


def p8_prepass(x, flop_per_in_byte):
    if (flop_per_in_byte is None or P8_PREPASS_MIN_FLOP_PER_BYTE <= 0 or flop_per_in_byte < P8_PREPASS_MIN_FLOP_PER_BYTE or not BF16_SPLIT or isinstance(x, P8)
            or torch.is_grad_enabled() or not x.is_cuda or x.shape[1] % 8 != 0 or x.shape[0] * (x.shape[1] // 8) * x.shape[2] * 16 >= (1 << 32)):
        return x
    return to_p8(x)


def conv_y_channels(c_out, act):
    return c_out // 2 if act in (ACT_GATE, ACT_WN_RES_SKIP) else c_out


def conv_desc(B, c_in, t_in, c_out, k, stride=1, dilation=1, pad_left=None, pad_mode=PAD_REFLECT, t_out=None, act=ACT_NONE, causal=True,
              k1=0, dilation2=0, c_out_pad=None, split_rows=0):
    if pad_left is None:
        t_o, padding_total, _ = conv_out_len(t_in, k, stride, dilation)
        pad_left = padding_total if causal else padding_total - padding_total // 2
        if t_out is None:
            t_out = t_o
    if t_out is None:
        raise ValueError("t_out required with explicit pad_left")
    d = ConvDesc()
    d.x_bs, d.x_cs = c_in * t_in, t_in
    d.y_bs, d.y_cs = conv_y_channels(c_out, act) * t_out, t_out
    d.B, d.C_in, d.T_in, d.C_out, d.C_out_pad, d.T_out = B, c_in, t_in, c_out, (pad32(c_out) if c_out_pad is None else c_out_pad), t_out
    d.K, d.stride, d.dilation, d.pad_left, d.pad_mode = k, stride, dilation, pad_left, pad_mode
    d.n_phase, d.y_tstride, d.act, d.w_batched, d.w_bs = 1, 1, act, 0, 0
    d.K1, d.dilation2, d.split_rows = k1, dilation2, split_rows
    d.pw_split = 1 if (BF16_SPLIT and PW_SPLIT and (k == 1 or (PW_TAPS and k == 4 and stride == 2))) else 0
    d.keep_tile160 = 0 if K1_COLUMN_TILES else 1
    return d


def conv1d(x, w_packed, c_out, k, bias=None, stride=1, dilation=1, pad_left=None, pad_mode=PAD_REFLECT,
           t_out=None, alpha_in=None, alpha_out=None, res=None, act=ACT_NONE, out=None, causal=True,
           alpha_y2=None, want_y=True, w_k1=None, bias_k1=None, w_split=None, k1=0, dilation2=0, skip_acc=None, gate_cond=None):
    x_p8 = x if isinstance(x, P8) else None
    if x_p8 is not None:
        B, c_in, t_in = x_p8.shape
    else:
        if not (x.is_cuda and x.dtype == torch.float32 and x.dim() == 3 and x.stride(2) == 1):
            x = _dev(x, "x")
        B, c_in, t_in = x.shape
    dev_ = x_p8.planes.device if x_p8 is not None else x.device
    d = conv_desc(B, c_in, t_in, c_out, k, stride, dilation, pad_left, pad_mode, t_out, act, causal, k1, dilation2,
                  w_packed.shape[-1] if w_packed is not None else None,
                  getattr(w_split, "split_rows", 0))
    t_out, c_y = d.T_out, conv_y_channels(c_out, act)
    if out is None and want_y:
        out = torch.empty(B, c_y, t_out, device=dev_, dtype=torch.float32)
    y2 = torch.empty(B, c_out, t_out, device=dev_, dtype=torch.float32) if alpha_y2 is not None else None
    if act == ACT_WN_RES_SKIP:
        assert skip_acc is not None and skip_acc.is_contiguous() and skip_acc.shape == out.shape and alpha_y2 is None
        y2 = skip_acc
    res = _dev(res, "res")
    d.bias = bias.data_ptr() if bias is not None else None
    if x_p8 is not None:
        d.x, d.x_p8, d.x_p8_plane_bytes = None, x_p8.planes.data_ptr(), x_p8.plane_bytes
    else:
        d.x = x.data_ptr()
        d.x_bs, d.x_cs = x.stride(0), x.stride(1)
    d.w = w_packed.data_ptr() if w_packed is not None else w_split.data_ptr()
    d.alpha_in = alpha_in.data_ptr() if alpha_in is not None else None
    d.alpha_out = alpha_out.data_ptr() if alpha_out is not None else None
    d.res = res.data_ptr() if res is not None else None
    d.y = out.data_ptr() if out is not None else None
    d.y2 = y2.data_ptr() if y2 is not None else None
    d.alpha_y2 = alpha_y2.data_ptr() if alpha_y2 is not None else None
    d.w_k1 = w_k1.data_ptr() if w_k1 is not None else None
    d.bias_k1 = bias_k1.data_ptr() if bias_k1 is not None else None
    d.w_split = w_split.data_ptr() if w_split is not None else None
    if out is not None and (out.stride(0), out.stride(1)) != (d.y_bs, d.y_cs) and out.shape[0] * out.shape[1] > 1:
        assert out.stride(2) == 1 and y2 is None and res is None and out.shape == (B, c_y, t_out)
        d.y_bs, d.y_cs = out.stride(0), out.stride(1)
    if gate_cond is not None:
        if not (gate_cond.is_cuda and gate_cond.dtype == torch.float32 and gate_cond.dim() == 2 and gate_cond.shape == (B, c_out)
                and (gate_cond.stride(1) == 1 or c_out == 1)):
            raise ValueError(f"gate_cond must be a float32 GPU tensor (B={B}, c_out={c_out}) with contiguous rows, "
                             f"got {tuple(gate_cond.shape)} {gate_cond.dtype} {gate_cond.device}")
        d.gate_cond, d.gate_cond_bs = gate_cond.data_ptr(), gate_cond.stride(0)
    _launch_conv(d, "fac_conv1d_fwd")
    return (out, y2) if alpha_y2 is not None else out


STREAM_FOLD = True
SKINNY_MAX_COLS = 640


def convtr_desc(B, c_in, t_in, c_out, stride, c_out_pad, causal=True, has_history=False, rows=False, split=False):
    t_cols = t_in - 1 if has_history else t_in
    t_total = t_cols * stride
    d = ConvDesc()
    d.x_bs, d.x_cs = c_in * t_in, t_in
    d.y_bs, d.y_cs = c_out * t_total, t_total
    d.B, d.C_in, d.T_in, d.C_out, d.C_out_pad, d.T_out = B, c_in, t_in, c_out, c_out_pad, t_cols
    d.K, d.stride, d.dilation, d.pad_left, d.pad_mode = 2, 1, 1, (0 if has_history else 1), PAD_ZERO
    d.n_phase, d.y_tstride, d.act, d.w_batched, d.w_bs = stride, stride, ACT_NONE, 0, 0
    d.phase_shift = 0 if causal else stride - stride // 2
    if rows or split:
        if not causal or has_history:
            raise _lib.FacodecHipError("the all-phases ConvTranspose1d launch is causal and offline only")
        d.n_phase, d.y_tstride, d.phase_shift, d.row_phases = 1, 1, 0, stride
        d.pw_split = 1 if (BF16_SPLIT and PW_SPLIT and PW_TAPS and not split and stride == 2) else 0
    return d


def conv_transpose1d(x, w_packed, c_out, stride, bias=None, alpha_in=None, out=None, alpha_y2=None, causal=True,
                     has_history=False):
    x_p8 = x if isinstance(x, P8) else None
    if x_p8 is not None:
        assert not has_history
        B, c_in, t_in = x_p8.shape
    else:
        if not (has_history and x.is_cuda and x.dtype == torch.float32 and x.stride(2) == 1):
            x = _dev(x, "x")
        B, c_in, t_in = x.shape
    dev_ = x_p8.planes.device if x_p8 is not None else x.device
    if has_history:
        assert causal
    split_rows = isinstance(w_packed, tuple)
    d = convtr_desc(B, c_in, t_in, c_out, stride, w_packed[1] if split_rows else w_packed.shape[-1], causal, has_history,
                    not split_rows and w_packed.dim() == 3, split_rows)
    if out is None:
        out = torch.empty(B, c_out, d.T_out * stride, device=dev_, dtype=torch.float32)
    d.bias = bias.data_ptr() if bias is not None else None
    if x_p8 is not None:
        d.x, d.x_p8, d.x_p8_plane_bytes = None, x_p8.planes.data_ptr(), x_p8.plane_bytes
    else:
        d.x = x.data_ptr()
        d.x_bs, d.x_cs = x.stride(0), x.stride(1)
    if split_rows:
        d.w, d.w_split = None, w_packed[0].data_ptr()
    else:
        d.w = w_packed.data_ptr()
    d.alpha_in = alpha_in.data_ptr() if alpha_in is not None else None
    d.alpha_out, d.res, d.y = None, None, out.data_ptr()
    y2 = torch.empty_like(out) if alpha_y2 is not None else None
    d.y2 = y2.data_ptr() if y2 is not None else None
    d.alpha_y2 = alpha_y2.data_ptr() if alpha_y2 is not None else None
    _launch_conv(d, "fac_conv1d_fwd(convtr)")
    return (out, y2) if alpha_y2 is not None else out


FLAT_TRAIN = True
PW_SPLIT = os.environ.get("FAC_PW_SPLIT", "1") != "0"
PW_TAPS = True
K1_COLUMN_TILES = True


def pack_conv_for(layout, v, g, stride=1, k1=0, scale=None):
    if layout in (W_FP32, W_FP32_PW_TAPS):
        return pack_conv_weight(v, g, scale=scale), None
    if layout == W_GEMM_STRIDED:
        return None, pack_gemm_weight_split(v, g, in_stride=stride, scale=scale)
# ... 1531 lines not shown
```

include/facodec_hip.h:

```cpp
#ifndef FACODEC_HIP_H
#define FACODEC_HIP_H

#include <stdint.h>

#ifdef __cplusplus
extern "C" {
#endif

typedef void* fac_stream_t;

#define FAC_OK 0
#define FAC_ERR_ARG (-1)
#define FAC_ERR_LAUNCH (-2)

#define FAC_PAD_ZERO 0
#define FAC_PAD_REFLECT 1

#define FAC_ACT_NONE 0
#define FAC_ACT_TANH 1
#define FAC_ACT_MISH 2
#define FAC_ACT_LOG_MEL 3
#define FAC_ACT_GATE 4
#define FAC_ACT_WN_RES_SKIP 5

int fac_version(void);
const char* fac_last_error(void);


int fac_wn_scale(const float* v, const float* g, float* scale, int n_slices, int slice_len,
                 fac_stream_t stream);

int fac_pack_conv_w(const float* v, const float* scale, float* packed, int C_out, int C_in,
                    int K, int C_out_pad, fac_stream_t stream);

int fac_pack_convtr_w(const float* v, const float* scale, float* packed, int C_in, int C_out,
                      int stride, int C_out_pad, fac_stream_t stream);

static inline int fac_convtr_rows(int C_out, int stride) {
  const int cpt = 128 / stride;
  return ((C_out + cpt - 1) / cpt) * 128;
}
int fac_pack_convtr_w_rows(const float* v, const float* scale, float* packed, int C_in, int C_out, int stride,
                           fac_stream_t stream);

#define FAC_CONV_WS_BYTES (32ll << 20)

typedef struct fac_conv_desc {
  const float* x;
  const float* w;
  const float* bias;
  const float* alpha_in;
  const float* alpha_out;
  const float* res;
  float* y;
  float* y2;
  const float* alpha_y2;
  const float* w_k1;
  const float* bias_k1;
  int64_t x_bs, x_cs;
  int64_t y_bs, y_cs;
  int32_t B, C_in, T_in, C_out, C_out_pad;
  int32_t T_out;
  int32_t K, stride, dilation, pad_left, pad_mode;
  int32_t n_phase;
  int32_t y_tstride;
  int32_t phase_shift;
  int32_t act;
  int32_t w_batched;
  int64_t w_bs;
  void* ws;
  int64_t ws_bytes;
  const void* w_split;
  int32_t K1, dilation2;
  int32_t row_phases;
  const void* x_p8;
  int64_t x_p8_plane_bytes;
  void* y2_p8;
  int64_t y2_p8_plane_bytes;
  int32_t pw_split;
  int32_t split_rows;
  const float* gate_cond;
  int64_t gate_cond_bs;
  int32_t keep_tile160;
} fac_conv_desc;

int fac_conv1d_fwd(const fac_conv_desc* d, fac_stream_t stream);
int fac_to_p8(const float* x, const float* alpha, void* out, int B, int C, int T, fac_stream_t stream);
int64_t fac_conv_w_split_bytes(int C_out, int C_in, int K);
int64_t fac_conv_w_split_rows_bytes(int C_out, int C_in, int K, int rows);
int fac_pack_conv_w_split_rows(const float* v, const float* scale, void* out, int C_out, int C_in, int K, int rows, fac_stream_t stream);
int fac_pack_conv_w_split(const float* v, const float* scale, void* out, int C_out, int C_in, int K,
                          fac_stream_t stream);
int64_t fac_conv_w_split2_bytes(int C_out, int C_in, int K, int K1);
int fac_pack_conv_w_split2(const float* v, const float* scale, void* out, int C_out, int C_in, int K, int K1, fac_stream_t stream);
int64_t fac_gemm_w_split_bytes(int R, int C_in, int K, int in_stride);
int fac_pack_gemm_w_split(const float* v, int64_t row_stride, int64_t ci_stride, int64_t k_stride, const float* row_scale, void* out,
                          int R, int C_in, int K, int in_stride, fac_stream_t stream);
int fac_conv1d_variant(const fac_conv_desc* d, char* name, int name_len);

int fac_snake_fwd(const float* x, const float* alpha, float* y, int B, int C, int T,
                  fac_stream_t stream);


int fac_lstm_to_time_major(const float* x, float* xT, int B, int H, int T, fac_stream_t stream);
int fac_lstm_from_time_major(const float* yT, const float* skip, const float* alpha, float* out, int B, int H, int T,
                             fac_stream_t stream);
int fac_pack_lstm_whh(const float* w_hh, float* packed, int H, fac_stream_t stream);
int fac_lstm_layer_fwd(const float* pre, const float* whh_packed, float* yT, float* c, int T,
                       int H, int BP, fac_stream_t stream);
int fac_lstm_layer_fwd_from(const float* pre, const float* whh_packed, float* yT, float* c, int T,
                            int H, int BP, int64_t step0, fac_stream_t stream);
int fac_lstm_layer_fwd_train(const float* pre, const float* whh_packed, float* yT, float* c, float* gates_save,
                             float* c_save, int T, int H, int BP, int64_t step0, fac_stream_t stream);
int fac_lstm_gate_bwd(const float* dy_t, const float* rec, const float* gates_t, const float* c_t, const float* c_prev,
                      float* dc, float* dgates_t, int H, int BP, int64_t rs, int first, fac_stream_t stream);
int fac_pack_lstm_whh_t(const float* w_hh, float* packed, int H, fac_stream_t stream);
int fac_lstm_layer_bwd(const float* dyT, const float* whh_t_packed, const float* gates, const float* cs, float* dgates, float* scratch,
                       int T, int H, int BP, fac_stream_t stream);

int fac_lstm_persist_ok(int H, int B);
int fac_lstm_persist_stream_ok(fac_stream_t stream);
int fac_pack_lstm_whh16(const float* w_hh, float* packed, int H, int transposed, fac_stream_t stream);
int fac_lstm_layer_fwd_persist(const float* pre, const float* whh16, float* hfrag, float* yT, float* gates_save, float* c_save,
                               int T, int H, int B, int BP, fac_stream_t stream);
int fac_lstm_layer_bwd_persist(const float* dyT, const float* whh16t, const float* gates, const float* cs, float* dgates,
                               float* scratch, int T, int H, int B, int BP, fac_stream_t stream);
int fac_lstm_persist_split_ok(int H, int B);
int fac_lstm_persist_timeouts(void);
int fac_lstm_persist_arm(fac_stream_t stream);
int fac_lstm_abort_flag(float* dst, fac_stream_t stream);
int fac_mask_flags_if(float* flags, int n, const float* poison, fac_stream_t stream);
int fac_pack_lstm_whh_split(const float* w_hh, void* packed, int H, fac_stream_t stream);
int fac_lstm_layer_fwd_persist_split(const float* pre, const void* wsplit, void* hsplit, float* yT, int T, int H, int B, int BP,
                                     fac_stream_t stream);
int fac_tanh_bwd(const float* y, const float* dy, float* dx, int64_t n, fac_stream_t stream);
int fac_pair_bwd(const float* a, const float* b, float* da, int64_t n, int mode, float eps, float scale, int accumulate,
                 fac_stream_t stream);
int fac_spec_power_bwd(const float* spec, const float* dout, float* dspec, int B, int F, int n_frames, int power,
                       fac_stream_t stream);
int fac_stft_frames_bwd(const float* dframes, float* dwave, int B, int T, int n_win, int n_frames, int hop, int pad,
                        int n_off, fac_stream_t stream);
int fac_vq_latent_bwd(const float* z_e, const float* codebook, const int64_t* codes, int64_t codes_bs, const float* d_zst,
                      const float* wc, float* d_ze, float* z_st, int B, int T, fac_stream_t stream);
int fac_vq_codebook_grad(const float* z_e, const float* codebook, const int64_t* codes, int64_t codes_bs, const float* wb,
                         float* dcb, int B, int T, int Kc, int accumulate, fac_stream_t stream);
int fac_layernorm_c_affine_bwd(const float* x, const float* style, const float* dout, float* dx, float* dstyle, float* stats,
                               int B, int C, int T, fac_stream_t stream);
int fac_rows_fma(const float* a, const float* w, const float* c, float* out, int B, int64_t per, float sign,
                 fac_stream_t stream);
int fac_grad_norm_clip(const float* g, int64_t n, float max_norm, float* scratch, float* norm_out, fac_stream_t stream);
int fac_adamw_step(float* p, const float* g, float* m, float* v, int64_t n, float lr, float beta1, float beta2, float eps,
                   float weight_decay, int64_t step, const float* clip, fac_stream_t stream);
int fac_adamw_step_masked(float* p, const float* g, float* m, float* v, int64_t n, const int64_t* offsets, int n_params,
                          const float* flags, int32_t* steps, float* bc, float lr, float beta1, float beta2, float eps,
                          float weight_decay, const float* clip, fac_stream_t stream);
int fac_gather_copy(const void* const* src, void* const* dst, const int64_t* n, int count, fac_stream_t stream);
int fac_gate_bwd(const float* a, const float* d, float* da, int B, int C, int T, fac_stream_t stream);
int fac_mish_fwd(const float* x, float* y, int64_t n, fac_stream_t stream);
int fac_mish_bwd(const float* x, const float* d, float* dx, int64_t n, fac_stream_t stream);
int fac_glu_bwd(const float* a, const float* d, float* da, int B, int C, int T, fac_stream_t stream);
int fac_mul_scaled(const float* a, const float* b, float* out, float scale, int64_t n, fac_stream_t stream);
int fac_embed_sum_bwd(const float* dx, const int64_t* codes, float* dtables, int B, int n_tab, int n_codes, int code_row0, int V,
                      int E, int T, fac_stream_t stream);
int fac_gate_bwd_cond(const float* a, const float* g, int64_t g_bs, const float* d, float* da, float* dcond, int64_t dcond_bs,
                      int B, int C, int T, fac_stream_t stream);
int fac_masked_mean_bwd(const float* dout, const float* mask, float* dx, int B, int C, int T, fac_stream_t stream);
int fac_attention_probs(const float* q, const float* k, const float* mask, float* P, int B, int H, int dk, int T,
                        fac_stream_t stream);
int fac_attention_pv(const float* P, const float* v, float* o, int B, int H, int dk, int T, fac_stream_t stream);
int fac_attention_bwd_pv(const float* P_used, const float* v, const float* dO, float* dv, float* dP, int B, int H, int dk,
                         int T, fac_stream_t stream);
int fac_attention_bwd_qk(const float* P, float* dP, const float* q, const float* k, const float* mask, float* dq, float* dk_,
                         int B, int H, int dk, int T, fac_stream_t stream);
int fac_aa_snakebeta_bwd(const float* x, const float* alpha_log, const float* beta_log, const float* filter12, const float* dy,
                         float* dx, float* dalpha, float* dbeta, float* scratch, int B, int C, int T, fac_stream_t stream);
// ... 328 lines not shown
```

Measured before the change: 1273 audio-s/s.

## Fuse k=1 residual-unit tail into bf16-split k=7 conv kernel for 64-channel blocks

```diff
diff --git a/facodec_amd/_lib.py b/facodec_amd/_lib.py
--- a/facodec_amd/_lib.py
+++ b/facodec_amd/_lib.py
@@ -29,6 +29,7 @@
         ("pw_split", C.c_int32), ("split_rows", C.c_int32),
         ("gate_cond", _p), ("gate_cond_bs", _i64),
         ("keep_tile160", C.c_int32),
+        ("w_k1_split", _p),
     ]
 
 
@@ -147,6 +148,8 @@
     "fac_pack_conv_w_split": (_i, [_p, _p, _p, _i, _i, _i, _p]),
     "fac_conv_w_split_rows_bytes": (_i64, [_i, _i, _i, _i]),
     "fac_pack_conv_w_split_rows": (_i, [_p, _p, _p, _i, _i, _i, _i, _p]),
+    "fac_pw_w_split_bytes": (_i64, [_i]),
+    "fac_pack_pw_w_split": (_i, [_p, _p, _p, _i, _p]),
     "fac_flip_transpose_w": (_i, [_p, _p, _p, _i, _i, _i, _p]),
     "fac_prep_begin": (_i, []),
     "fac_prep_set_phase": (_i, [_i]),
diff --git a/facodec_amd/build.py b/facodec_amd/build.py
--- a/facodec_amd/build.py
+++ b/facodec_amd/build.py
@@ -9,7 +9,7 @@
 LIB = os.path.join(HERE, "libfacodec_hip%s.so" % ("_" + TAG if TAG else ""))
 OBJDIR = "build" + ("_" + TAG if TAG else "")
 SOURCES = ["conv1d_api.hip", "conv1d_tile_128x128.hip", "conv1d_tile_96x128.hip", "conv1d_tile_64x128.hip",
-           "conv1d_tile_32x256.hip", "conv1d_tile_128x32.hip", "conv1d_tile_128x256.hip", "conv1d_fused_ru.hip", "conv1d_narrow.hip", "conv1d_pw.hip", "conv1d_pw_split.hip", "conv1d_skinny.hip", "conv1d_bsplit.hip", "conv1d_bsplit96.hip", "conv1d_gemm_split.hip", "conv1d_bsplit2.hip", "conv1d_bwd.hip", "conv1d_wgrad_split.hip", "conv1d_wgrad_k1.hip", "train_misc.hip", "optim.hip", "train_quant.hip", "train_pred.hip", "train_disc.hip", "train_redecoder.hip", "pack.hip", "prep_batch.hip", "lstm.hip", "lstm_persist.hip", "vq.hip", "vq_decode.hip", "bitpack.hip", "misc.hip", "attention_stream.hip", "attention_tiled.hip","ragged.hip", "resample.hip", "loudness.hip", "metrics.hip", "stream_pool.hip", "plc.hip", "jdc.hip", "rccl_arena.hip"]
+           "conv1d_tile_32x256.hip", "conv1d_tile_128x32.hip", "conv1d_tile_128x256.hip", "conv1d_fused_ru.hip", "conv1d_narrow.hip", "conv1d_pw.hip", "conv1d_pw_split.hip", "conv1d_skinny.hip", "conv1d_bsplit.hip", "conv1d_bsplit96.hip", "conv1d_bsplit_ru.hip", "conv1d_gemm_split.hip", "conv1d_bsplit2.hip", "conv1d_bwd.hip", "conv1d_wgrad_split.hip", "conv1d_wgrad_k1.hip", "train_misc.hip", "optim.hip", "train_quant.hip", "train_pred.hip", "train_disc.hip", "train_redecoder.hip", "pack.hip", "prep_batch.hip", "lstm.hip", "lstm_persist.hip", "vq.hip", "vq_decode.hip", "bitpack.hip", "misc.hip", "attention_stream.hip", "attention_tiled.hip","ragged.hip", "resample.hip", "loudness.hip", "metrics.hip", "stream_pool.hip", "plc.hip", "jdc.hip", "rccl_arena.hip"]
 FLAGS = ["--offload-arch=gfx950", "-O3", "-std=c++17", "-fPIC", "-ffp-contract=off",
          "-Wno-unused-result"] + os.environ.get("FAC_EXTRA_FLAGS", "").split()
 
diff --git a/facodec_amd/convplan.py b/facodec_amd/convplan.py
--- a/facodec_amd/convplan.py
+++ b/facodec_amd/convplan.py
@@ -1,7 +1,7 @@
 from collections import namedtuple
 
 __all__ = ["ConvPlan", "ConvTrPlan", "plan_conv", "plan_convtr", "plan_gemm", "tile_rows", "gemm_split_ok", "gemm_split_strided_ok", "split2_ok",
-           "pw_taps_ok", "pw_split_tail_ok", "convtr_split_ok", "convtr_rows_ok", "flat_strided_ok", "flat_convtr_ok", "W_FP32", "W_TAPS",
+           "pw_taps_ok", "pw_split_tail_ok", "ru_split_fused_ok", "convtr_split_ok", "convtr_rows_ok", "flat_strided_ok", "flat_convtr_ok", "W_FP32", "W_TAPS",
            "W_GEMM", "W_GEMM_STRIDED", "W_SPLIT2", "W_FP32_PW_TAPS", "PER_CLIP", "FLAT_STRIDED", "FLAT_STRIDE1", "TR_POLYPHASE", "TR_ROWS",
            "TR_ROWS_SPLIT", "TR_ROWS_PW_TAPS", "TR_FLAT"]
 
@@ -77,6 +77,13 @@
     return 96 if (sw.BF16_SPLIT and not grad and k == 7 and c_out in sw.BS_ROWS96 and c_in % 8 == 0) else 64
 
 
+def ru_split_fused_ok(c, dilation, batch, t):
+    sw = _sw()
+    if not (sw.BF16_SPLIT and c in sw.RU_SPLIT_FUSED and c == 64 and batch * t > 640 and c * t < (1 << 30)):
+        return False
+    return tile_rows(c, c, 7) == 64 and 2 * ((256 + 6 * dilation + 63) // 64) <= 12
+
+
 def plan_conv(c_out, c_in, k, stride, dilation, batch, t_in, t_out, *, k1=0, alpha_in=False, plain=True, res=False,
               causal_reflect=False, grad=True, c_out_mult16=True, split_k=(1, 3, 5, 7), floor_k=(3, 5), tail="pw_split",
               pw_taps=True, split2=False, flat_infer=False, flat_stride1=False, flat_train=None):
diff --git a/facodec_amd/csrc/conv1d_api.hip b/facodec_amd/csrc/conv1d_api.hip
--- a/facodec_amd/csrc/conv1d_api.hip
+++ b/facodec_amd/csrc/conv1d_api.hip
@@ -66,6 +66,7 @@
   a.x = d->x; a.w = d->w; a.bias = d->bias; a.alpha_in = d->alpha_in; a.alpha_out = d->alpha_out;
   a.res = d->res; a.y = d->y; a.y2 = d->y2; a.alpha2 = d->alpha_y2;
   a.w1 = d->w_k1; a.bias1 = d->bias_k1;
+  a.w1_split = static_cast<const unsigned char*>(d->w_k1_split);
   a.x_p8 = reinterpret_cast<const unsigned char*>(d->x_p8); a.x_p8_ps = d->x_p8_plane_bytes;
   a.y2_p8 = reinterpret_cast<unsigned char*>(d->y2_p8); a.y2_p8_ps = d->y2_p8_plane_bytes;
   FAC_REQUIRE(!d->y2_p8 || d->alpha_y2, "conv1d: y2_p8 needs alpha_y2");
@@ -114,6 +115,18 @@
     FAC_REQUIRE(d->w && !d->w_k1 && !d->x_p8 && !conv_two_level(a) && conv_skinny_ok(a, d->ws, d->ws_bytes),
                 "conv1d: FAC_ACT_GATE / FAC_ACT_WN_RES_SKIP exist only for few-column launches (B * T_out <= 640) with a workspace");
     k = CK_SKINNY;
+    return FAC_OK;
+  }
+  if (d->w_k1_split) {
+    FAC_REQUIRE(d->w_split && !d->w_k1 && d->K == 7 && d->C_out == 64 && (d->split_rows == 0 || d->split_rows == 64) &&
+                    conv_bsplit_ru_ok(a) && !conv_cin1_ok(a),
+                "conv1d: w_k1_split needs a stride-1 k = 7 launch on w_split (64-row tiles) with fp32 input, C_in == C_out == 64, alpha_out, "
+                "res, no act and more than 640 columns (K=%d stride=%d C_in=%d C_out=%d split_rows=%d columns=%lld)",
+                d->K, d->stride, d->C_in, d->C_out, d->split_rows, (long long)d->B * d->T_out);
+    a.w = reinterpret_cast<const float*>(d->w_split);
+    a.gflat = 0;
+    a.grt = 0;
+    k = CK_BSPLIT;
     return FAC_OK;
   }
   if (d->w_k1) { k = CK_FUSED_RU; return FAC_OK; }
@@ -186,7 +199,7 @@
     case CK_128x160: return conv_dispatch_128x160(a, s);
     case CK_NARROW: return conv_dispatch_narrow(a, s);
     case CK_SKINNY: return conv_dispatch_skinny(a, d->ws, d->ws_bytes, s);
-    case CK_BSPLIT: return conv_dispatch_bsplit(a, s);
+    case CK_BSPLIT: return a.w1_split ? conv_dispatch_bsplit_ru(a, s) : conv_dispatch_bsplit(a, s);
     case CK_CIN1: return conv_dispatch_cin1(a, s);
     case CK_THIN: return conv_dispatch_thin(a, d->ws, s);
     case CK_PW: return conv_dispatch_pw(a, s);
@@ -224,7 +237,10 @@
       snprintf(name, name_len, conv_skinny_single_launch(a) ? "conv1d_gemv_kernel (single launch, <=4 columns)"
                                                             : "conv1d_skinny_kernel (split reduction, <=640 columns)");
       break;
-    case CK_BSPLIT: snprintf(name, name_len, "conv1d_bsplit_kernel<%d> 64x256 (bf16x3 split, fp32-grade)", a.K); break;
+    case CK_BSPLIT:
+      if (a.w1_split) snprintf(name, name_len, "conv1d_bsplit_kernel<%d,RU> %dx256 (bf16x3 split, k=1 tail fused, fp32-grade)", a.K, a.C_out);
+      else snprintf(name, name_len, "conv1d_bsplit_kernel<%d> 64x256 (bf16x3 split, fp32-grade)", a.K);
+      break;
     case CK_CIN1: snprintf(name, name_len, "conv1d_cin1_kernel (VALU, C_in=1, store stream)"); break;
     case CK_THIN: snprintf(name, name_len, "conv1d_thin_kernel (VALU, C_out<=8, split channels)"); break;
     case CK_PW: snprintf(name, name_len, "conv1d_pw_kernel (k=1 streaming, W in LDS)"); break;
diff --git a/facodec_amd/csrc/conv1d_bsplit_kernel.h b/facodec_amd/csrc/conv1d_bsplit_kernel.h
--- a/facodec_amd/csrc/conv1d_bsplit_kernel.h
+++ b/facodec_amd/csrc/conv1d_bsplit_kernel.h
@@ -32,7 +32,7 @@
   return __int_as_float(__builtin_amdgcn_ds_bpermute(((lane & 48) + j) << 2, __float_as_int(mine)));
 }
 
-template <int KT, int G, int NMW, int NSW, int MB = 2>
+template <int KT, int G, int NMW, int NSW, int MB = 2, bool RU = false>
 __global__ __launch_bounds__((NMW + NSW) * 64, (NMW + NSW) / 4) void conv1d_bsplit_kernel(ConvArgs a) {
   constexpr int NB = 2;
   constexpr int CO = 32 * MB;
@@ -72,6 +72,9 @@
   };
   const bool overlap = a.persist != 0;
   unsigned char* epi_base = sm + (overlap ? STG : 0);
+  constexpr int EPI_BYTES = CO * (BS_TT + 4) * 4;
+  unsigned char* ru_tab = nullptr;
+  if constexpr (RU) ru_tab = sm + (overlap ? STG + (STG > EPI_BYTES ? STG : EPI_BYTES) : (2 * STG > EPI_BYTES ? 2 * STG : EPI_BYTES));
   auto walk = [&](auto role) {
   constexpr int ROLE = decltype(role)::value;
   constexpr bool STAGING = ROLE != 0;
@@ -469,8 +472,155 @@
           tile[(m * 32 + (r & 3) + 8 * (r >> 2) + 4 * kq) * EP + n0 + n * 32 + l31] = acc[m][n][r];
   }
   }
+  bf16x8 ruA[RU ? MB : 1][3];
+  auto ru_load_a = [&](const unsigned char* wl, int s) {
+#pragma unroll
+    for (int m = 0; m < (RU ? MB : 1); ++m)
+#pragma unroll
+      for (int p = 0; p < 3; ++p) ruA[m][p] = *reinterpret_cast<const bf16x8*>(wl + ((s * MB + m) * 3 + p) * 1024);
+  };
+  if constexpr (RU) {
+    const KArgP e = fresh_args();
+    if constexpr (STAGING) {
+      const int c = tid - NMW * 64;
+      if (c < CO) {
+        float4* tab = reinterpret_cast<float4*>(ru_tab);
+        const float al = e->alpha_out[c], a2 = e->y2 ? e->alpha2[c] : 0.f;
+        tab[c] = make_float4(e->bias ? e->bias[c] : 0.f, al, snake_inv(al), 0.f);
+        tab[CO + c] = make_float4(e->bias1 ? e->bias1[c] : 0.f, a2, e->y2 ? snake_inv(a2) : 0.f, 0.f);
+      }
+    } else {
+      asm volatile("" ::: "memory");
+      __builtin_amdgcn_sched_barrier(0);
+      int ln = lane;
+      asm volatile("" : "+v"(ln));
+      ru_load_a(e->w1_split + ln * 16, 0);
+    }
+  }
   __syncthreads();
 
+  if constexpr (RU) {
+    static_assert(!RU || (NMW + NSW == 8 && BS_TT == 256), "RU tail: eight waves of 32 columns");
+    auto keep_low = [&]() {
+      if constexpr (STAGING) asm volatile("" ::: FAC_XREGS48_CLOBBERS);
+    };
+    keep_low();
+    const KArgP e = fresh_args();
+    float* tile = reinterpret_cast<float*>(epi_base);
+    const float4* tab = reinterpret_cast<const float4*>(ru_tab);
+    constexpr int EP = BS_TT + 4;
+    constexpr int S16 = CO / 16;
+    int ln = lane;
+    asm volatile("" : "+v"(ln));
+    const int l31 = ln & 31, kq = ln >> 5;
+    const int col = wave * 32 + l31;
+    const bool ok = t0 + col < e->T_out;
+    const int last = e->T_out - 1 - (t0 + wave * 32);
+    const unsigned char* wl = e->w1_split + ln * 16;
+    float* tp = tile + 8 * kq * EP + col;
+    const float4* tp1 = tab + 8 * kq;
+#pragma unroll 1
+    for (int s = 0; s < S16; ++s) {
+      keep_low();
+#pragma unroll
+      for (int j = 0; j < 8; ++j) {
+        const float4 c = tp1[16 * s + j];
+        float v = tp[(16 * s + j) * EP] + c.x;
+        v = snake_apply(v, c.y, c.z);
+        v = v + 0.f;
+        tp[(16 * s + j) * EP] = v;
+      }
+    }
+    keep_low();
+    if constexpr (STAGING) ru_load_a(wl, 0);
+    unsigned ycs4 = (unsigned)e->y_cs * 4u;
+    asm volatile("" : "+s"(ycs4));
+    const unsigned voff = (unsigned)(4 * kq) * ycs4 + (unsigned)l31 * 4u;
+    const unsigned roff = (unsigned)(4 * kq) * ycs4 + (unsigned)(l31 < last ? l31 : (last > 0 ? last : 0)) * 4u;
+    const long long obase = (long long)b * e->y_bs + t0 + wave * 32;
+    const unsigned char* rg = reinterpret_cast<const unsigned char*>(e->res + obase);
+    unsigned char* yg = e->y ? reinterpret_cast<unsigned char*>(e->y + obase) : nullptr;
+    unsigned char* y2g = e->y2 ? reinterpret_cast<unsigned char*>(e->y2 + obase) : nullptr;
+    f32x16 acc[MB];
+#pragma unroll
+    for (int m = 0; m < MB; ++m)
+#pragma unroll
+      for (int r = 0; r < 16; ++r) acc[m][r] = 0.f;
+    float rv[MB][16];
+#pragma unroll
+    for (int s = 0; s < S16; ++s) {
+      bf16x8 B[3];
+#pragma unroll
+      for (int j = 0; j < 8; ++j) {
+        __bf16 b0, b1, b2;
+        split3_scalar_sub(tp[(16 * s + j) * EP], b0, b1, b2);
+        B[0][j] = b0; B[1][j] = b1; B[2][j] = b2;
+        keep_low();
+      }
+#pragma unroll
+      for (int m = 0; m < MB; ++m) {
+        const bf16x8 A0 = ruA[m][0], A1 = ruA[m][1], A2 = ruA[m][2];
+        acc[m] = __builtin_amdgcn_mfma_f32_32x32x16_bf16(A1, B[1], acc[m], 0, 0, 0);
+        acc[m] = __builtin_amdgcn_mfma_f32_32x32x16_bf16(A2, B[0], acc[m], 0, 0, 0);
+        acc[m] = __builtin_amdgcn_mfma_f32_32x32x16_bf16(A0, B[2], acc[m], 0, 0, 0);
+        acc[m] = __builtin_amdgcn_mfma_f32_32x32x16_bf16(A1, B[0], acc[m], 0, 0, 0);
+        acc[m] = __builtin_amdgcn_mfma_f32_32x32x16_bf16(A0, B[1], acc[m], 0, 0, 0);
+        acc[m] = __builtin_amdgcn_mfma_f32_32x32x16_bf16(A0, B[0], acc[m], 0, 0, 0);
+      }
+      __builtin_amdgcn_sched_barrier(0);
+      if (s + 1 < S16) {
+        ru_load_a(wl, s + 1);
+      } else {
+#pragma unroll
+        for (int m = 0; m < MB; ++m)
+#pragma unroll
+          for (int r = 0; r < 16; ++r) {
+            const unsigned row = m * 32 + (r & 3) + 8 * (r >> 2);
+            rv[m][r] = last >= 0 ? *reinterpret_cast<const float*>(rg + (roff + row * ycs4)) : 0.f;
+          }
+      }
+      __builtin_amdgcn_sched_barrier(0);
+      keep_low();
+    }
+    const float4* tab2 = tab + CO + 4 * kq;
+    float* mine = tile + 4 * kq * EP + col;
+    const bool sy = yg != nullptr && ok;
+#pragma unroll
+    for (int m = 0; m < MB; ++m) {
+#pragma unroll
+      for (int q = 0; q < 4; ++q) {
+#pragma unroll
+        for (int i = 0; i < 4; ++i) {
+          const int r = 4 * q + i;
+          const float v = acc[m][r] + tab2[m * 32 + i + 8 * q].x;
+          acc[m][r] = v + rv[m][r];
+        }
+        if (sy) {
+#pragma unroll
+          for (int i = 0; i < 4; ++i) *reinterpret_cast<float*>(yg + (voff + (unsigned)(m * 32 + i + 8 * q) * ycs4)) = acc[m][4 * q + i];
+        }
+        if (y2g) {
+#pragma unroll
+          for (int i = 0; i < 4; ++i) mine[(m * 32 + i + 8 * q) * EP] = acc[m][4 * q + i];
+        }
+        __builtin_amdgcn_sched_barrier(0);
+        keep_low();
+      }
+    }
+    if (y2g && ok) {
+#pragma unroll 1
+      for (int g = 0; g < 4 * MB; ++g) {
+        keep_low();
+#pragma unroll
+        for (int i = 0; i < 4; ++i) {
+          const int row = 8 * g + i;
+          const float4 c = tab2[row];
+          *reinterpret_cast<float*>(y2g + (voff + (unsigned)row * ycs4)) = snake_apply(mine[row * EP], c.y, c.z);
+        }
+      }
+    }
+    keep_low();
+  } else
   {
     const KArgP e = fresh_args();
     const float* tile = reinterpret_cast<const float*>(epi_base);
@@ -549,12 +699,13 @@
   }
 }
 
-template <int KT, int G, int NMW, int NSW, int MB = 2>
+template <int KT, int G, int NMW, int NSW, int MB = 2, bool RU = false>
 static int bsplit_launch(ConvArgs& a, hipStream_t s) {
   constexpr int H = bs_slots(KT, G), TT = 64 * NMW, CO = 32 * MB;
   a.XW = TT + (H / G - 1) * a.dil;
   const size_t stg = (size_t)3 * H * CO * 16 + (size_t)48 * G * a.XW;
   const size_t epi = (size_t)CO * (TT + 4) * sizeof(float);
+  constexpr size_t tab = RU ? (size_t)2 * CO * 16 : 0;
   a.n_t_tiles = (a.T_out + TT - 1) / TT;
   const long long n_wg = (long long)a.n_t_tiles * ((a.C_out + CO - 1) / CO) * a.B;
   if (n_wg > 0x7fffffffll) {
@@ -564,13 +715,13 @@
   const int n_chunks = (a.C_in + 8 * G - 1) / (8 * G);
   int cus = device_cus() & ~7;
   a.persist = (NMW == 4 && a.x_p8 == nullptr && n_chunks % 2 == 0 && cus >= 8 && n_wg > cus &&
-               stg + (stg > epi ? stg : epi) <= FAC_LDS_MAX) ? 1 : 0;
-  size_t lds = a.persist ? stg + (stg > epi ? stg : epi) : (2 * stg > epi ? 2 * stg : epi);
+               stg + (stg > epi ? stg : epi) + tab <= FAC_LDS_MAX) ? 1 : 0;
+  size_t lds = (a.persist ? stg + (stg > epi ? stg : epi) : (2 * stg > epi ? 2 * stg : epi)) + tab;
   if (lds > FAC_LDS_MAX) {
     set_error("conv1d(bf16 split): tile needs %zu B of LDS (dil=%d)", lds, a.dil);
     return FAC_ERR_ARG;
   }
-  constexpr auto kern = conv1d_bsplit_kernel<KT, G, NMW, NSW, MB>;
+  constexpr auto kern = conv1d_bsplit_kernel<KT, G, NMW, NSW, MB, RU>;
   allow_dynamic_lds<kern>();
   a.n_tiles = (int)n_wg;
   hipLaunchKernelGGL(kern, dim3((unsigned)(a.persist ? cus : n_wg)), dim3((NMW + NSW) * 64), lds, s, a);
diff --git a/facodec_amd/csrc/conv1d_bsplit_ru.hip b/facodec_amd/csrc/conv1d_bsplit_ru.hip
--- /dev/null
+++ b/facodec_amd/csrc/conv1d_bsplit_ru.hip
@@ -0,0 +1,14 @@
+#include "conv1d_bsplit_kernel.h"
+
+namespace fac {
+
+bool conv_bsplit_ru_ok(const ConvArgs& a) {
+  if (!(a.w1_split && a.alpha_out && a.res && a.act == FAC_ACT_NONE && !a.x_p8 && !a.y2_p8 && a.C_in == a.C_out && a.rp == 1 &&
+        !conv_two_level(a) && a.T_in >= a.T_out && a.y_cs > 0 && a.y_cs * (long long)a.C_out < (1ll << 30)))
+    return false;
+  return a.K == 7 && a.C_out == BS_CO && conv_bsplit_ok(a) && bs_group(a.C_in) == 2;
+}
+
+int conv_dispatch_bsplit_ru(ConvArgs& a, hipStream_t s) { return bsplit_launch<7, 2, 4, BS_NSW_WIDE, 2, true>(a, s); }
+
+}
diff --git a/facodec_amd/csrc/conv1d_mfma.h b/facodec_amd/csrc/conv1d_mfma.h
--- a/facodec_amd/csrc/conv1d_mfma.h
+++ b/facodec_amd/csrc/conv1d_mfma.h
@@ -43,6 +43,7 @@
   int rp;
   const float* gate_cond;
   long long gate_cond_bs;
+  const unsigned char* w1_split;
 };
 
 __host__ __device__ inline int conv_max_tap_offset(const ConvArgs& a) {
@@ -621,6 +622,8 @@
 bool conv_bsplit96_ok(const ConvArgs& a);
 bool conv_bsplit96_p8_ok(const ConvArgs& a);
 int conv_dispatch_bsplit96(ConvArgs& a, hipStream_t s);
+bool conv_bsplit_ru_ok(const ConvArgs& a);
+int conv_dispatch_bsplit_ru(ConvArgs& a, hipStream_t s);
 bool conv_pws_ok(const ConvArgs& a);
 int conv_dispatch_pws(ConvArgs& a, hipStream_t s);
 bool conv_pwt_ok(const ConvArgs& a);
diff --git a/facodec_amd/csrc/inflight_regs.h b/facodec_amd/csrc/inflight_regs.h
--- a/facodec_amd/csrc/inflight_regs.h
+++ b/facodec_amd/csrc/inflight_regs.h
@@ -12,3 +12,7 @@
   M(11, 227) M(12, 228) M(13, 229) M(14, 230) M(15, 231) M(16, 232) M(17, 233) M(18, 234) M(19, 235) M(20, 236) M(21, 237) M(22, 238) M(23, 239) \
   M(24, 240) M(25, 241) M(26, 242) M(27, 243) M(28, 244) M(29, 245) M(30, 246) M(31, 247) M(32, 248) M(33, 249) M(34, 250) M(35, 251) M(36, 252) \
   M(37, 253) M(38, 254) M(39, 255)
+#define FAC_XREGS48_CLOBBERS                                                                                                        \
+  "v208", "v209", "v210", "v211", "v212", "v213", "v214", "v215", "v216", "v217", "v218", "v219", "v220", "v221", "v222", "v223",   \
+  "v224", "v225", "v226", "v227", "v228", "v229", "v230", "v231", "v232", "v233", "v234", "v235", "v236", "v237", "v238", "v239",   \
+  "v240", "v241", "v242", "v243", "v244", "v245", "v246", "v247", "v248", "v249", "v250", "v251", "v252", "v253", "v254", "v255"
diff --git a/facodec_amd/csrc/misc.hip b/facodec_amd/csrc/misc.hip
--- a/facodec_amd/csrc/misc.hip
+++ b/facodec_amd/csrc/misc.hip
@@ -593,7 +593,7 @@
 
 using namespace fac;
 
-extern "C" int fac_version(void) { return 5; }
+extern "C" int fac_version(void) { return 6; }
 extern "C" const char* fac_last_error(void) { return fac::g_err; }
 
 #define EW_LAUNCH(kern, n, ...)                                                         \
diff --git a/facodec_amd/csrc/pack.hip b/facodec_amd/csrc/pack.hip
--- a/facodec_amd/csrc/pack.hip
+++ b/facodec_amd/csrc/pack.hip
@@ -143,6 +143,35 @@
   flip_transpose_w_body(v, scale, out, C_out, C_in, K, n, blockIdx.x, gridDim.x);
 }
 
+__device__ __forceinline__ void pack_pw_split_body(const float* __restrict__ v, const float* __restrict__ scale,
+                                                   unsigned char* __restrict__ out, int C, long long n, int vb, int vg) {
+  const int NB = C / 32;
+  for (long long i = (long long)vb * 256 + threadIdx.x; i < n; i += (long long)vg * 256) {
+    const int ln = (int)(i & 63), rest = (int)(i >> 6);
+    const int mb = rest % NB, s = rest / NB;
+    const int co = 32 * mb + (ln & 31);
+    const int ci0 = 16 * s + 8 * (ln >> 5);
+    bf16x8 h, m, l;
+#pragma unroll
+    for (int j = 0; j < 8; ++j) {
+      float w = v[(long long)co * C + ci0 + j];
+      if (scale) w = __fmul_rn(w, scale[co]);
+      __bf16 a0, a1, a2;
+      split3(w, a0, a1, a2);
+      h[j] = a0; m[j] = a1; l[j] = a2;
+    }
+    unsigned char* dst = out + ((size_t)(s * NB + mb) * 3) * 1024 + ln * 16;
+    *reinterpret_cast<bf16x8*>(dst) = h;
+    *reinterpret_cast<bf16x8*>(dst + 1024) = m;
+    *reinterpret_cast<bf16x8*>(dst + 2048) = l;
+  }
+}
+
+__global__ __launch_bounds__(256) void pack_pw_split_kernel(const float* __restrict__ v, const float* __restrict__ scale,
+                                                            unsigned char* __restrict__ out, int C, long long n) {
+  pack_pw_split_body(v, scale, out, C, n, blockIdx.x, gridDim.x);
+}
+
 __global__ __launch_bounds__(256) void pack_batch_kernel(const PrepJob* __restrict__ jobs, const int* __restrict__ first, int njobs) {
   __shared__ float sm[32 * 33];
   const int j = prep_find_job(first, njobs, blockIdx.x);
@@ -157,6 +186,7 @@
     case PK_CONVTR: pack_convtr_body(a, b, o, J.i[0], J.i[1], J.i[2], J.i[3], vb % J.i[4], vb / J.i[4], sm); break;
     case PK_CONVTR_ROWS: pack_convtr_rows_body(a, b, o, J.i[0], J.i[1], J.i[2], J.i[3], J.n, vb, J.nblocks); break;
     case PK_FLIP_T: flip_transpose_w_body(a, b, o, J.i[0], J.i[1], J.i[2], J.n, vb, J.nblocks); break;
+    case PK_PW_SPLIT: pack_pw_split_body(a, b, static_cast<unsigned char*>(J.out), J.i[0], J.n, vb, J.nblocks); break;
     default: break;
   }
 }
@@ -267,6 +297,23 @@
   return check_launch("flip_transpose_w");
 }
 
+extern "C" int64_t fac_pw_w_split_bytes(int C) { return (C > 0 && C % 32 == 0) ? (int64_t)6 * C * C : -1; }
+
+extern "C" int fac_pack_pw_w_split(const float* v, const float* scale, void* out, int C, fac_stream_t stream) {
+  using namespace fac;
+  FAC_REQUIRE(v && out && C > 0 && C % 32 == 0, "pack_pw_w_split: C must be a positive multiple of 32 (C=%d)", C);
+  const long long n = (long long)(C / 16) * (C / 32) * 64;
+  const int blocks = prep_blocks(n);
+  if (prep_recording()) {
+    PrepJob j{}; j.a = v; j.b = scale; j.out = out; j.kind = PK_PW_SPLIT; j.nblocks = blocks; j.n = n;
+    j.i[0] = C;
+    return prep_record(PU_PACK, j);
+  }
+  hipLaunchKernelGGL(pack_pw_split_kernel, dim3(blocks), dim3(256), 0, (hipStream_t)stream, v, scale,
+                     static_cast<unsigned char*>(out), C, n);
+  return check_launch("pack_pw_w_split");
+}
+
 extern "C" int fac_pack_lstm_whh(const float* w_hh, float* packed, int H, fac_stream_t stream) {
   using namespace fac;
   FAC_REQUIRE(w_hh && packed && H > 0 && H % 8 == 0, "pack_lstm_whh: H must be a multiple of 8");
diff --git a/facodec_amd/csrc/prep_batch.h b/facodec_amd/csrc/prep_batch.h
--- a/facodec_amd/csrc/prep_batch.h
+++ b/facodec_amd/csrc/prep_batch.h
@@ -21,7 +21,8 @@
   PK_CONV_SPLIT,
   PK_GEMM_SPLIT,
   PK_CONV_SPLIT2,
-  PK_CONV_BWD
+  PK_CONV_BWD,
+  PK_PW_SPLIT
 };
 
 bool prep_recording();
diff --git a/facodec_amd/dac_model.py b/facodec_amd/dac_model.py
--- a/facodec_amd/dac_model.py
+++ b/facodec_amd/dac_model.py
@@ -23,7 +23,7 @@
     def alpha_in(self):
         return self.block[0].flat()
 
-    def run(self, x, x_act, alpha_next=None, want_raw=True, edge=None):
+    def run(self, x, x_act, alpha_next=None, want_raw=True, edge=None, keep_two_launches=False):
         b = self.block
         k7, k1 = b[1], b[3]
         streaming = ops.BF16_SPLIT and x.shape[0] * ((x.shape[-1] + 31) // 32) >= 8192
@@ -33,6 +33,14 @@
                                      alpha_out=b[2].flat(), res=x, w_k1=k1.w.packed(), bias_k1=k1.w.bias,
                                      alpha_y2=alpha_next, want_y=want_raw or alpha_next is None, causal=k7.causal)
             return return_pair if alpha_next is not None else (return_pair, None)
+        if (streaming and not keep_two_launches and x_act.shape[-1] == x.shape[-1]
+                and ops.ru_split_fused_ok(k7.w.c_out, k7.dilation, x.shape[0], x.shape[-1])):
+            write_edge(k7, x_act, edge)
+            c = k7.w.c_out
+            pair = ops.conv1d(x_act, None, c, 7, bias=k7.w.bias, dilation=k7.dilation, pad_mode=k7.pad_mode, alpha_out=b[2].flat(),
+                              res=x, w_split=k7.w.packed_split(ops.tile_rows(c, c, 7)), w_k1_split=k1.w.packed_k1_split(),
+                              bias_k1=k1.w.bias, alpha_y2=alpha_next, want_y=want_raw or alpha_next is None, causal=k7.causal)
+            return pair if alpha_next is not None else (pair, None)
         h = b[1].run(x_act, alpha_out=b[2].flat(), edge=edge)
         if h.shape[-1] != x.shape[-1]:
             pad = (x.shape[-1] - h.shape[-1]) // 2
diff --git a/facodec_amd/layers.py b/facodec_amd/layers.py
--- a/facodec_amd/layers.py
+++ b/facodec_amd/layers.py
@@ -30,6 +30,7 @@
         self._split = None
         self._rows = None
         self._rows_split = None
+        self._k1_split = None
         self.freeze_packed = False
 
     def _vg(self):
@@ -59,9 +60,13 @@
     def packed_split(self, rows=64):
         return self._cached("_split", ops.pack_conv_weight_split, rows=rows)
 
+    def packed_k1_split(self):
+        return self._cached("_k1_split", ops.pack_pw_weight_split)
+
     def _apply(self, fn, *a, **kw):
         self._packed = None
         self._split = None
+        self._k1_split = None
         self._rows = None
         self._rows_split = None
         return super()._apply(fn, *a, **kw)
diff --git a/facodec_amd/ops.py b/facodec_amd/ops.py
--- a/facodec_amd/ops.py
+++ b/facodec_amd/ops.py
@@ -197,6 +197,7 @@
 
 BF16_SPLIT = True
 BS_ROWS96 = (96,)
+RU_SPLIT_FUSED = (64,)
 
 
 def set_conv_profile(p):
@@ -302,7 +303,7 @@
     d.ws, d.ws_bytes = ws.data_ptr(), CONV_WS_BYTES
     if _FLOPS is not None or _PROFILE is not None:
         flops = 2.0 * d.B * d.n_phase * max(1, d.row_phases) * d.C_out * d.T_out * d.C_in * d.K
-        if d.w_k1:
+        if d.w_k1 or d.w_k1_split:
             flops += 2.0 * d.B * d.C_out * d.T_out * d.C_out
     if _FLOPS is not None:
         _FLOPS.add(_FLOP_KEY, flops)
@@ -403,6 +404,22 @@
     return out
 
 
+@prepared
+def pack_pw_weight_split(v, g=None, out=None, scale=None):
+    v = _dev(v, "weight")
+    c_out, c_in, k = v.shape
+    lib = _lib.load()
+    nbytes = lib.fac_pw_w_split_bytes(c_out) if (k == 1 and c_in == c_out) else -1
+    if nbytes < 0:
+        raise _lib.FacodecHipError("pack_pw_weight_split: needs (C, C, 1) weights with C %% 32 == 0, got %s" % (tuple(v.shape),))
+    if scale is None and g is not None:
+        scale = wn_scale(v, g)
+    if out is None:
+        out = torch.empty(nbytes, device=v.device, dtype=torch.uint8)
+    _lib.check(lib.fac_pack_pw_w_split(_ptr(v), _ptr(scale), out.data_ptr(), c_out, _stream()), "fac_pack_pw_w_split")
+    return out
+
+
 def conv_out_len(t_in, k, stride, dilation):
     k_eff = (k - 1) * dilation + 1
     padding_total = k_eff - stride
@@ -477,7 +494,8 @@
 
 def conv1d(x, w_packed, c_out, k, bias=None, stride=1, dilation=1, pad_left=None, pad_mode=PAD_REFLECT,
            t_out=None, alpha_in=None, alpha_out=None, res=None, act=ACT_NONE, out=None, causal=True,
-           alpha_y2=None, want_y=True, w_k1=None, bias_k1=None, w_split=None, k1=0, dilation2=0, skip_acc=None, gate_cond=None):
+           alpha_y2=None, want_y=True, w_k1=None, bias_k1=None, w_split=None, k1=0, dilation2=0, skip_acc=None, gate_cond=None,
+           w_k1_split=None):
     x_p8 = x if isinstance(x, P8) else None
     if x_p8 is not None:
         B, c_in, t_in = x_p8.shape
@@ -513,6 +531,7 @@
     d.w_k1 = w_k1.data_ptr() if w_k1 is not None else None
     d.bias_k1 = bias_k1.data_ptr() if bias_k1 is not None else None
     d.w_split = w_split.data_ptr() if w_split is not None else None
+    d.w_k1_split = w_k1_split.data_ptr() if w_k1_split is not None else None
     if out is not None and (out.stride(0), out.stride(1)) != (d.y_bs, d.y_cs) and out.shape[0] * out.shape[1] > 1:
         assert out.stride(2) == 1 and y2 is None and res is None and out.shape == (B, c_y, t_out)
         d.y_bs, d.y_cs = out.stride(0), out.stride(1)
diff --git a/include/facodec_hip.h b/include/facodec_hip.h
--- a/include/facodec_hip.h
+++ b/include/facodec_hip.h
@@ -82,6 +82,7 @@
   const float* gate_cond;
   int64_t gate_cond_bs;
   int32_t keep_tile160;
+  const void* w_k1_split;
 } fac_conv_desc;
 
 int fac_conv1d_fwd(const fac_conv_desc* d, fac_stream_t stream);
@@ -91,6 +92,8 @@
 int fac_pack_conv_w_split_rows(const float* v, const float* scale, void* out, int C_out, int C_in, int K, int rows, fac_stream_t stream);
 int fac_pack_conv_w_split(const float* v, const float* scale, void* out, int C_out, int C_in, int K,
                           fac_stream_t stream);
+int64_t fac_pw_w_split_bytes(int C);
+int fac_pack_pw_w_split(const float* v, const float* scale, void* out, int C, fac_stream_t stream);
 int64_t fac_conv_w_split2_bytes(int C_out, int C_in, int K, int K1);
 int fac_pack_conv_w_split2(const float* v, const float* scale, void* out, int C_out, int C_in, int K, int K1, fac_stream_t stream);
 int64_t fac_gemm_w_split_bytes(int R, int C_in, int K, int in_stride);
```

Result: no change. 1280 audio-s/s, median of 6 (+0.6%).
